# ugonfor/DGQ

Measured on AMD Instinct MI355X. Metric: UNet denoise steps/sec @ SD1.4 512^2 W4A8 g16, higher is better.
Workload: dtype int8 (W4A8 MFMA, int32 accumulate; fp32 between layers); 1 GPU; SD v1.4 UNet W4A8 g=16 (time-aware, log2 softmax real-time δ, start-peak), DDIM 50-step schedule, 512x512 (64x64 latents), CFG pair per step per GPU; config_id=c2, prompts_per_gpu=1, batch_per_gpu=2, parallelism=replicas x1 (no collectives)

## Files before the change

### dgq_amd/csrc/conv_f32w.hip

```cpp
#include "quant_common.h"

typedef float v16f __attribute__((ext_vector_type(16)));

struct ConvF32Params {
    const void* x;
    const float* w;
    const float* bias;
    const float* pre_scale;
    const float* pre_shift;
    int pre_act;
    void* y;
    void* y2;
    int ldy2;
    float* gn_partial;
    int x_dtype, y_dtype;
    int B, H, W, C, kh, kw, stride, pad, Ho, Wo, N, K, M, ldy;
};

__device__ __forceinline__ float ld_any(const void* p, int dtype, int64_t i);
__device__ __forceinline__ float ld_pre(const ConvF32Params& p, int b, int64_t pix, int c) {
    float v = ld_any(p.x, p.x_dtype, pix * p.C + c);
    if (p.pre_scale) v = v * p.pre_scale[(int64_t)b * p.C + c] + p.pre_shift[(int64_t)b * p.C + c];
    if (p.pre_act == 1) v = dgq_silu(v);
    return v;
}

__device__ __forceinline__ void store_any(void* p, int dtype, int64_t i, float v) {
    if (dtype == DGQ_F16) reinterpret_cast<__half*>(p)[i] = __float2half(v);
    else if (dtype == DGQ_BF16) reinterpret_cast<__hip_bfloat16*>(p)[i] = __float2bfloat16(v);
    else reinterpret_cast<float*>(p)[i] = v;
}
__device__ __forceinline__ float ld_any(const void* p, int dtype, int64_t i) {
    if (dtype == DGQ_F16) return __half2float(reinterpret_cast<const __half*>(p)[i]);
    if (dtype == DGQ_BF16) return __bfloat162float(reinterpret_cast<const __hip_bfloat16*>(p)[i]);
    return reinterpret_cast<const float*>(p)[i];
}

#define CF_BM 64
#define CF_BN 64
#define CF_BK 16
#define CF_LD (CF_BK + 1)

__global__ __launch_bounds__(256) void conv_f32w_kernel(ConvF32Params p) {
    __shared__ float As[CF_BM][CF_LD];
    __shared__ float Bs[CF_BN][CF_LD];
    const int tid = threadIdx.x, lane = tid & 63, wid = tid >> 6;
    const int m0 = blockIdx.y * CF_BM, n0 = blockIdx.x * CF_BN;
    const int wm = (wid >> 1) * 32, wn = (wid & 1) * 32;
    const int srow = tid >> 2, sk = (tid & 3) * 4;
    const int am = m0 + srow;
    int ab = 0, aho = 0, awo = 0;
    if (am < p.M) {
        const int L = p.Ho * p.Wo;
        ab = am / L;
        const int l = am - ab * L;
        aho = l / p.Wo;
        awo = l - aho * p.Wo;
    }
    v16f acc;
#pragma unroll
    for (int r = 0; r < 16; ++r) acc[r] = 0.0f;
    for (int k0 = 0; k0 < p.K; k0 += CF_BK) {
#pragma unroll
        for (int j = 0; j < 4; ++j) {
            const int k = k0 + sk + j;
            float a = 0.0f, b = 0.0f;
            if (k < p.K) {
                if (am < p.M) {
                    const int tap = k / p.C, c = k - tap * p.C;
                    const int dh = tap / p.kw, dw = tap - dh * p.kw;
                    const int hi = aho * p.stride - p.pad + dh, wi = awo * p.stride - p.pad + dw;
                    if (hi >= 0 && hi < p.H && wi >= 0 && wi < p.W)
                        a = ld_pre(p, ab, ((int64_t)ab * p.H + hi) * p.W + wi, c);
                }
                if (n0 + srow < p.N) b = p.w[(int64_t)(n0 + srow) * p.K + k];
            }
            As[srow][sk + j] = a;
            Bs[srow][sk + j] = b;
        }
        __syncthreads();
#pragma unroll
        for (int kk = 0; kk < CF_BK; kk += 2) {
            const float av = As[wm + (lane & 31)][kk + (lane >> 5)];
            const float bv = Bs[wn + (lane & 31)][kk + (lane >> 5)];
            acc = __builtin_amdgcn_mfma_f32_32x32x2f32(av, bv, acc, 0, 0, 0);
        }
        __syncthreads();
    }
    const int n = n0 + wn + (lane & 31);
    if (n >= p.N) return;
    const float bias = p.bias ? p.bias[n] : 0.0f;
#pragma unroll
    for (int r = 0; r < 16; ++r) {
        const int m = m0 + wm + (r & 3) + 8 * (r >> 2) + 4 * (lane >> 5);
        if (m >= p.M) continue;
        const float v = acc[r] + bias;
        store_any(p.y, p.y_dtype, (int64_t)m * p.ldy + n, v);
        if (p.y2) store_any(p.y2, p.y_dtype, (int64_t)m * p.ldy2 + n, v);
    }
    if (p.gn_partial) {
#pragma unroll
        for (int blk = 0; blk < 2; ++blk) {
            float val[8], sum = 0.0f;
#pragma unroll
            for (int q = 0; q < 8; ++q) {
                float v = acc[blk * 8 + q] + bias;
                if (p.y_dtype == DGQ_F16) v = __half2float(__float2half(v));
                else if (p.y_dtype == DGQ_BF16) v = __bfloat162float(__float2bfloat16(v));
                val[q] = v;
                sum += v;
            }
            float mean = sum * 0.125f, m2 = 0.0f;
#pragma unroll
            for (int q = 0; q < 8; ++q) m2 += (val[q] - mean) * (val[q] - mean);
            const float om = __shfl_xor(mean, 32, 64), o2 = __shfl_xor(m2, 32, 64);
            const float dd = om - mean;
            m2 = m2 + o2 + dd * dd * 4.0f;
            mean = 0.5f * (mean + om);
            const int mb = m0 + wm + blk * 16;
            if ((lane >> 5) == 0 && mb < p.M) {
                float* q2 = p.gn_partial + ((int64_t)(mb >> 4) * p.N + n) * 2;
                q2[0] = mean; q2[1] = m2;
            }
        }
    }
}

template <int NMAX>
__global__ __launch_bounds__(256) void conv_f32w_smalln_kernel(ConvF32Params p) {
    const int lane = threadIdx.x & 63;
    const int m = blockIdx.x * 4 + (threadIdx.x >> 6);
    if (m >= p.M) return;
    const int L = p.Ho * p.Wo;
    const int b = m / L, l = m - b * L;
    const int ho = l / p.Wo, wo = l - ho * p.Wo;
    float acc[NMAX];
#pragma unroll
    for (int n = 0; n < NMAX; ++n) acc[n] = 0.0f;
    const bool vec = (p.C & 3) == 0 && (reinterpret_cast<uintptr_t>(p.x) & 15) == 0 &&
                     (reinterpret_cast<uintptr_t>(p.w) & 15) == 0 &&
                     (!p.pre_scale || (((reinterpret_cast<uintptr_t>(p.pre_scale) | reinterpret_cast<uintptr_t>(p.pre_shift)) & 15) == 0));
    if (vec) {
        const int c4n = p.C >> 2, units = p.kh * p.kw * c4n;
        constexpr int UB = NMAX <= 4 ? 4 : 2;
        for (int u0 = lane; u0 < units; u0 += 64 * UB) {
            float4 v[UB], sc[UB], sh[UB], w4[UB][NMAX];
            bool inb[UB];
#pragma unroll
            for (int j = 0; j < UB; ++j) {
                const int u = min(u0 + 64 * j, units - 1);
                const int tap = u / c4n, c = (u - tap * c4n) << 2;
                const int dh = tap / p.kw, dw = tap - dh * p.kw;
                const int hi = ho * p.stride - p.pad + dh, wi = wo * p.stride - p.pad + dw;
                inb[j] = (u0 + 64 * j < units) && hi >= 0 && hi < p.H && wi >= 0 && wi < p.W;
                const int hc = min(max(hi, 0), p.H - 1), wc = min(max(wi, 0), p.W - 1);
                const int64_t xi = (((int64_t)b * p.H + hc) * p.W + wc) * p.C + c;
                float t4[4];
                if (p.x_dtype == DGQ_F32) load4<float>(reinterpret_cast<const float*>(p.x) + xi, t4);
                else if (p.x_dtype == DGQ_BF16) load4<__hip_bfloat16>(reinterpret_cast<const __hip_bfloat16*>(p.x) + xi, t4);
                else load4<__half>(reinterpret_cast<const __half*>(p.x) + xi, t4);
                v[j] = make_float4(t4[0], t4[1], t4[2], t4[3]);
                if (p.pre_scale) {
                    sc[j] = *reinterpret_cast<const float4*>(p.pre_scale + (int64_t)b * p.C + c);
                    sh[j] = *reinterpret_cast<const float4*>(p.pre_shift + (int64_t)b * p.C + c);
                }
#pragma unroll
                for (int n = 0; n < NMAX; ++n)
                    if (n < p.N) w4[j][n] = *reinterpret_cast<const float4*>(p.w + (int64_t)n * p.K + (int64_t)tap * p.C + c);
            }
#pragma unroll
            for (int j = 0; j < UB; ++j) {
                float4 t = v[j];
                if (p.pre_scale) {
                    t.x = t.x * sc[j].x + sh[j].x; t.y = t.y * sc[j].y + sh[j].y; t.z = t.z * sc[j].z + sh[j].z; t.w = t.w * sc[j].w + sh[j].w;
                }
                if (p.pre_act == 1) { t.x = dgq_silu(t.x); t.y = dgq_silu(t.y); t.z = dgq_silu(t.z); t.w = dgq_silu(t.w); }
                if (!inb[j]) t = make_float4(0.0f, 0.0f, 0.0f, 0.0f);
#pragma unroll
                for (int n = 0; n < NMAX; ++n)
                    if (n < p.N) {
                        acc[n] = __builtin_fmaf(t.x, w4[j][n].x, acc[n]);
                        acc[n] = __builtin_fmaf(t.y, w4[j][n].y, acc[n]);
                        acc[n] = __builtin_fmaf(t.z, w4[j][n].z, acc[n]);
                        acc[n] = __builtin_fmaf(t.w, w4[j][n].w, acc[n]);
                    }
            }
        }
    } else
    for (int k = lane; k < p.K; k += 64) {
        const int tap = k / p.C, c = k - tap * p.C;
        const int dh = tap / p.kw, dw = tap - dh * p.kw;
        const int hi = ho * p.stride - p.pad + dh, wi = wo * p.stride - p.pad + dw;
        if (hi < 0 || hi >= p.H || wi < 0 || wi >= p.W) continue;
        const float a = ld_pre(p, b, ((int64_t)b * p.H + hi) * p.W + wi, c);
#pragma unroll
        for (int n = 0; n < NMAX; ++n)
            if (n < p.N) acc[n] = __builtin_fmaf(a, p.w[(int64_t)n * p.K + k], acc[n]);
    }
#pragma unroll
    for (int n = 0; n < NMAX; ++n) {
        float v = acc[n];
#pragma unroll
        for (int o = 32; o > 0; o >>= 1) v += __shfl_xor(v, o, 64);
        if (lane == 0 && n < p.N) {
            v += p.bias ? p.bias[n] : 0.0f;
            store_any(p.y, p.y_dtype, (int64_t)m * p.ldy + n, v);
            if (p.y2) store_any(p.y2, p.y_dtype, (int64_t)m * p.ldy2 + n, v);
        }
    }
}

extern "C" int dgq_conv2d_f32w(const void* x, int x_dtype, int B, int H, int W, int C, int kh, int kw, int stride, int pad,
                               const float* w, const float* bias, int N, void* y, int y_dtype, int ldy,
                               const float* pre_scale, const float* pre_shift, int pre_act, void* y2, int ldy2, float* gn_partial, void* stream) {
    DGQ_CHECK_ARG(x && w && y, "dgq_conv2d_f32w: null pointer");
    DGQ_CHECK_ARG(B > 0 && H > 0 && W > 0 && C > 0 && kh > 0 && kw > 0 && stride > 0 && pad >= 0 && N > 0, "dgq_conv2d_f32w: bad geometry");
    DGQ_CHECK_ARG((x_dtype == DGQ_F32 || x_dtype == DGQ_F16 || x_dtype == DGQ_BF16) && (y_dtype == DGQ_F32 || y_dtype == DGQ_F16 || y_dtype == DGQ_BF16),
                  "dgq_conv2d_f32w: unknown dtype");
    DGQ_CHECK_ARG((pre_scale == nullptr) == (pre_shift == nullptr) && (pre_act == 0 || pre_act == 1), "dgq_conv2d_f32w: bad prologue");
    ConvF32Params p;
    p.pre_scale = pre_scale; p.pre_shift = pre_shift; p.pre_act = pre_act;
    p.x = x; p.w = w; p.bias = bias; p.y = y; p.x_dtype = x_dtype; p.y_dtype = y_dtype;
    p.B = B; p.H = H; p.W = W; p.C = C; p.kh = kh; p.kw = kw; p.stride = stride; p.pad = pad;
    p.Ho = (H + 2 * pad - kh) / stride + 1; p.Wo = (W + 2 * pad - kw) / stride + 1;
    DGQ_CHECK_ARG(p.Ho > 0 && p.Wo > 0, "dgq_conv2d_f32w: empty output");
    p.N = N; p.K = kh * kw * C; p.M = B * p.Ho * p.Wo; p.ldy = ldy;
    DGQ_CHECK_ARG(ldy >= N && (!y2 || ldy2 >= N), "dgq_conv2d_f32w: ldy < N");
    p.y2 = y2; p.ldy2 = ldy2;
    DGQ_CHECK_ARG(!gn_partial || (p.M % 16 == 0 && N > 8), "dgq_conv2d_f32w: GroupNorm partials need M %% 16 == 0 and the tiled kernel (N > 8)");
    p.gn_partial = gn_partial;
    if (N <= 8) {
        if (N <= 4) hipLaunchKernelGGL(conv_f32w_smalln_kernel<4>, dim3((p.M + 3) / 4), dim3(256), 0, (hipStream_t)stream, p);
        else hipLaunchKernelGGL(conv_f32w_smalln_kernel<8>, dim3((p.M + 3) / 4), dim3(256), 0, (hipStream_t)stream, p);
        return dgq_launch_status("dgq_conv2d_f32w");
    }
    dim3 grid((N + CF_BN - 1) / CF_BN, (p.M + CF_BM - 1) / CF_BM);
    DGQ_CHECK_ARG(grid.y <= 65535, "dgq_conv2d_f32w: M = %d rows exceed the grid", p.M);
    hipLaunchKernelGGL(conv_f32w_kernel, grid, dim3(256), 0, (hipStream_t)stream, p);
    return dgq_launch_status("dgq_conv2d_f32w");
}
```

### dgq_amd/csrc/gemm_tile.h

```cpp
#pragma once
#include <atomic>
#include <cstdio>
#include <cstdlib>
#include <type_traits>
#include "dgq_common.h"
#include "gemm_device.h"
#include "gemm_flush.h"
#include "diag.h"

#define BK 128

typedef int v16i __attribute__((ext_vector_type(16)));
typedef float v16f __attribute__((ext_vector_type(16)));

struct GemmParams {
    const int8_t* codes;
    const float* rowsum;
    int rowsum_parts;
    int M, Kp, N;
    const uint8_t* wpacked;
    const float* cdelta;
    const uint8_t* cflush;
    const float* mdelta;
    const float* mzp;
    int L;
    float offset;
    const float* alpha;
    const float* zw;
    const float* gamma;
    const float* vn;
    void* y;
    int ldy;
    float* slab;
    int splits;
    int tiles_per_split;
    dgq_gemm_extra_t ex;
    dgq_gemm_conv_t cv;
    const float* ccoef;
    const uint8_t* wfrag;
    dgq_gemm_act_t act;
};

#define DGQ_GEMM_BATCH 8
struct GemmBatch {
    GemmParams p[DGQ_GEMM_BATCH];
    int n;
};

__device__ __forceinline__ void gemm_prefetch_params(const GemmParams& p) {
    asm volatile("" ::"s"(p.M), "s"(p.N), "s"(p.Kp), "s"(p.tiles_per_split), "s"(p.splits), "s"(p.codes), "s"(p.wpacked), "s"(p.rowsum),
                 "s"(p.rowsum_parts), "s"(p.alpha), "s"(p.zw), "s"(p.gamma), "s"(p.vn), "s"(p.cdelta), "s"(p.cflush), "s"(p.mdelta),
                 "s"(p.mzp), "s"(p.L), "s"(p.offset), "s"(p.y), "s"(p.ldy), "s"(p.slab), "s"(p.ex.residual), "s"(p.ex.ldr),
                 "s"(p.ex.res_div), "s"(p.ex.res_dtype), "s"(p.ex.fq_mode), "s"(p.ex.geglu), "s"(p.ex.gn_partial), "s"(p.wfrag), "s"(p.ex.y2));
}

template <bool PER_M>
__device__ __forceinline__ float dgq_epilogue(const GemmParams& p, float acc, int m, int n, float al, float zw, float ga,
                                              float vn) {
    float rs = 0.0f;
    for (int j = 0; j < p.rowsum_parts; ++j) rs += p.rowsum[(int64_t)j * p.M + m];
    if (PER_M) {
        const int li = m % p.L;
        const float md = p.mdelta[li], mz = p.mzp[li];
        return dgq_dequant<true>(acc, md, md * rs, md * (p.offset - mz), al, zw, ga, vn);
    }
    return dgq_dequant<false>(acc, 1.0f, rs, 0.0f, al, zw, ga, vn);
}

constexpr int gemm_stage_bytes(int wbits, int bm, int bn) { return bm * BK + bn * (wbits == 4 ? BK / 2 : BK); }
constexpr int gemm_waves_per_simd(int wbits, int bm, int bn, int nw, int nst) {
    const int per_block = nst * gemm_stage_bytes(wbits, bm, bn) + 6 * 1024;
    int o = (160 * 1024) / per_block;
    o = o > 5 ? 5 : (o < 1 ? 1 : o);
    const int w = o * nw / 4;
    return w > 8 ? 8 : w;
}

__device__ __forceinline__ float gload_f32(const float* q) {
    float v;
    asm volatile("global_load_dword %0, %1, off" : "=v"(v) : "v"(q) : "memory");
    return v;
}
__device__ __forceinline__ uint32_t gload_u8(const uint8_t* q) {
    uint32_t v;
    asm volatile("global_load_ubyte %0, %1, off" : "=v"(v) : "v"(q) : "memory");
    return v;
}
template <int N>
__device__ __forceinline__ void wait_vmcnt_lgkm0() {
    asm volatile("s_waitcnt vmcnt(%0) lgkmcnt(0)" ::"n"(N) : "memory");
}
template <int PER, int MAXT>
__device__ __forceinline__ void wait_ring(int tiles) {
    static_assert(PER * MAXT <= 63, "vmcnt is a 6-bit counter");
    if (tiles <= 0) wait_vmcnt_lgkm0<0>();
    else if (MAXT >= 1 && tiles == 1) wait_vmcnt_lgkm0<PER>();
    else if (MAXT >= 2 && tiles == 2) wait_vmcnt_lgkm0<PER * (MAXT >= 2 ? 2 : 0)>();
    else if (MAXT >= 3 && tiles == 3) wait_vmcnt_lgkm0<PER * (MAXT >= 3 ? 3 : 0)>();
    else wait_vmcnt_lgkm0<PER * (MAXT >= 4 ? 4 : 0)>();
}

struct GemmColRegs { float al, zw, ga, vn; };
template <bool PER_M>
__device__ __forceinline__ GemmColRegs gemm_cols_issue(const GemmParams& p, int n) {
    GemmColRegs c;
    c.al = gload_f32(p.alpha + n); c.zw = gload_f32(p.zw + n); c.ga = gload_f32(p.gamma + n);
    c.vn = 0.0f;
    if constexpr (PER_M) c.vn = gload_f32(p.vn + n);
    return c;
}
template <bool PER_M, int BN>
__device__ __forceinline__ void gemm_cols_commit(GemmColRegs& c, float* vcol, int tid, bool has_col) {
    if (PER_M) asm volatile("" : "+v"(c.al), "+v"(c.zw), "+v"(c.ga), "+v"(c.vn));
    else asm volatile("" : "+v"(c.al), "+v"(c.zw), "+v"(c.ga));
    __builtin_amdgcn_sched_barrier(0);
    if (has_col) {
        vcol[tid] = c.al; vcol[BN + tid] = c.zw; vcol[2 * BN + tid] = c.ga; vcol[3 * BN + tid] = c.vn;
    }
}
struct GemmFlushRegs { FlushRef x; float d, dn; uint32_t cf; };
template <typename Ref>
__device__ __forceinline__ GemmFlushRegs gemm_flush_issue(const GemmParams& p, int n_tab, int tid, Ref&& ref) {
    GemmFlushRegs f;
    f.x = ref(min(tid, n_tab - 1));
    f.d = gload_f32(p.cdelta + f.x.g); f.dn = gload_f32(p.cdelta + f.x.gn); f.cf = gload_u8(p.cflush + f.x.tl);
    return f;
}
template <int NT, typename Ref>
__device__ __forceinline__ void gemm_flush_commit(const GemmParams& p, GemmFlushRegs& f, float* ctab, int n_tab, int tid, Ref&& ref) {
    asm volatile("" : "+v"(f.d), "+v"(f.dn), "+v"(f.cf));
    __builtin_amdgcn_sched_barrier(0);
    if (tid < n_tab) ctab[tid] = flush_value(f.x, f.d, f.dn, f.cf);
    for (int e = tid + NT; e < n_tab; e += NT) ctab[e] = flush_entry(ref(e), p.cdelta, p.cflush);
}

template <bool BIASED, int TM, int TN>
__device__ __forceinline__ void gemm_flush(v16f (&accf)[TM][TN], const v16i (&ac)[TM][TN], float coef) {
    const float sc = __builtin_bit_cast(float, __builtin_amdgcn_readfirstlane(__builtin_bit_cast(int, coef)));
    if (sc != 0.0f) {
#pragma unroll
        for (int i = 0; i < TM; ++i)
#pragma unroll
            for (int j = 0; j < TN; ++j)
#pragma unroll
                for (int r = 0; r < 16; ++r) accf[i][j][r] = __builtin_fmaf(sc, dgq_total_to_float<BIASED>(ac[i][j][r]), accf[i][j][r]);
    }
}
template <int ACC0, int ACCS, int TM, int TN>
__device__ __forceinline__ void gemm_clear_totals(v16i (&acc)[ACCS][TM][TN]) {
#pragma unroll
    for (int a = 0; a < ACCS; ++a)
#pragma unroll
        for (int i = 0; i < TM; ++i)
#pragma unroll
            for (int j = 0; j < TN; ++j)
#pragma unroll
                for (int r = 0; r < 16; ++r) acc[a][i][j][r] = ACC0;
}


template <bool PER_M, typename TOut, int BM, int BN, int WVM, int WVN, int WVK, int LDS_CAP, int TM, int TN, bool TILED = false>
__device__ __forceinline__ void gemm_store_tile(const GemmParams& p, int zsplit, uint8_t* smem, const float* vtab, const float* vcol,
                                                int wid, int lane, int wave_m, int wave_n, int wave_k, int m0, int n0,
                                                const v16i (&acc0)[TM][TN], const v16f (&accf)[TM][TN] DGQ_DIAG_PARAM,
                                                int tiled_w = 0, int tiled_gn0 = 0) {
    static_assert(!TILED || (BM == 32 && WVM == 1 && WVK == 1), "tiled rows: one 32-row tile per workgroup");
    constexpr int NW = WVM * WVN * WVK;
    constexpr int WM = BM / WVM, WN = BN / WVN;
    static_assert(TM == WM / 32 && TN == WN / 32, "wave tile");
    const int lr = lane & 31, hh = lane >> 5;
    constexpr int EP_LD = WN + 4;
    constexpr int LPR = WN / 4;
    constexpr int RPP = 64 / LPR;
    constexpr int PASSES = WM / RPP / WVK;
    constexpr int EPH = (NW * WM * EP_LD * 4 <= LDS_CAP) ? 1 : 2;
    static_assert(EPH == 1 || (WVK == 1 && TM % 2 == 0 && PASSES % 2 == 0), "half-tile staging: whole MFMA row tiles per half");
    constexpr int HROWS = WM / EPH;
    constexpr int REGION = HROWS * EP_LD;
    static_assert(NW * REGION * 4 <= LDS_CAP, "epilogue staging must fit the LDS ring");
    float* ep_all = reinterpret_cast<float*>(smem);
    float* ep = ep_all + wid * REGION;
    auto stage_half = [&](int h) {
#pragma unroll
        for (int i = 0; i < TM / EPH; ++i)
#pragma unroll
            for (int j = 0; j < TN; ++j)
#pragma unroll
                for (int r = 0; r < 16; ++r) {
                    const int ti = h * (TM / EPH) + i;
                    ep[(i * 32 + (r & 3) + 8 * (r >> 2) + 4 * hh) * EP_LD + j * 32 + lr] = PER_M ? (float)acc0[ti][j][r] : accf[ti][j][r];
                }
        asm volatile("s_waitcnt lgkmcnt(0)" ::: "memory");
    };
    auto next_half = [&](int rr) {
        if (EPH == 2 && rr == PASSES / 2) {
            asm volatile("s_waitcnt lgkmcnt(0)" ::: "memory");
            stage_half(1);
        }
    };
    stage_half(0);
    if (WVK > 1) __builtin_amdgcn_s_barrier();
    DGQ_STAMP(8);
    const float* ep0 = ep_all + (wave_m * WVN + wave_n) * REGION;
    const float* ep1 = ep0 + (WVM * WVN) * REGION;
    const int c4 = (lane % LPR) * 4;
    const int lrow = lane / LPR;
    const int nb = n0 + wave_n * WN + c4;
    const bool vec_ok = (nb + 3 < p.N);
    auto tile_row = [&](int rr) { return wave_k * (WM / WVK) + rr * RPP + lrow; };
    auto row_m = [&](int row) { return TILED ? m0 + (row >> 3) * tiled_w + (row & 7) : m0 + wave_m * WM + row; };
    auto tile_val = [&](int row) {
        const int sr = (EPH == 2) ? (row & (HROWS - 1)) : row;
        float4 v = *reinterpret_cast<const float4*>(ep0 + sr * EP_LD + c4);
        if (WVK > 1) {
            const float4 u = *reinterpret_cast<const float4*>(ep1 + sr * EP_LD + c4);
            v.x += u.x; v.y += u.y; v.z += u.z; v.w += u.w;
        }
        return v;
    };
    if (p.splits > 1) {
        float* slab = p.slab + (int64_t)zsplit * p.M * p.N;
        const bool al16 = ((p.N & 3) == 0);
#pragma unroll 4
        for (int rr = 0; rr < PASSES; ++rr) {
            next_half(rr);
            const int row = tile_row(rr);
            const int m = row_m(row);
            if (m >= p.M || nb >= p.N) continue;
            const float4 v = tile_val(row);
            float* dst = slab + (int64_t)m * p.N + nb;
            if (vec_ok && al16) {
                *reinterpret_cast<float4*>(dst) = v;
            } else {
                const float e[4] = {v.x, v.y, v.z, v.w};
                for (int k = 0; k < 4 && nb + k < p.N; ++k) dst[k] = e[k];
            }
        }
        return;
    }
    TOut* y = reinterpret_cast<TOut*>(p.y);
    const float* vc = vcol + wave_n * WN + c4;
    const float4 al = *reinterpret_cast<const float4*>(vc);
    const float4 zw = *reinterpret_cast<const float4*>(vc + BN);
    const float4 ga = *reinterpret_cast<const float4*>(vc + 2 * BN);
    const float4 vn = *reinterpret_cast<const float4*>(vc + 3 * BN);
    if (p.ex.geglu) {
        const int ob = nb >> 1;
        const bool st2 = vec_ok && (p.ldy % 2 == 0) && ((reinterpret_cast<uintptr_t>(p.y) & 7) == 0);
#pragma unroll
        for (int rr = 0; rr < PASSES; ++rr) {
            next_half(rr);
            const int row = tile_row(rr);
            const int m = row_m(row);
            if (m >= p.M || nb >= p.N) continue;
            const float4 v = tile_val(row);
            const float* vr = vtab + wave_m * WM + row;
            const float r0 = vr[0], r1 = vr[BM], r2 = vr[2 * BM];
            const float a0 = dgq_dequant<PER_M>(v.x, r0, r1, r2, al.x, zw.x, ga.x, vn.x);
            const float g0 = dgq_dequant<PER_M>(v.y, r0, r1, r2, al.y, zw.y, ga.y, vn.y);
            const float a1 = dgq_dequant<PER_M>(v.z, r0, r1, r2, al.z, zw.z, ga.z, vn.z);
            const float g1 = dgq_dequant<PER_M>(v.w, r0, r1, r2, al.w, zw.w, ga.w, vn.w);
            const float o0 = dgq_geglu(a0, g0), o1 = dgq_geglu(a1, g1);
            TOut* dst = y + (int64_t)m * p.ldy + ob;
            if (st2) {
                if (sizeof(TOut) == 4) {
                    *reinterpret_cast<float2*>(dst) = make_float2(o0, o1);
                } else {
                    TOut t[2] = {dgq_from_float<TOut>(o0), dgq_from_float<TOut>(o1)};
                    *reinterpret_cast<uint32_t*>(dst) = *reinterpret_cast<const uint32_t*>(t);
                }
            } else {
                dst[0] = dgq_from_float<TOut>(o0);
                if (nb + 3 < p.N) dst[1] = dgq_from_float<TOut>(o1);
            }
        }
        return;
    }
    const bool st_vec = vec_ok && ((p.ldy * (int)sizeof(TOut)) % 16 == 0) &&
                        ((reinterpret_cast<uintptr_t>(p.y) & 15) == 0) && (sizeof(TOut) == 4 || (p.ldy & 3) == 0);
    const bool st_vec2 = vec_ok && ((p.ex.ldy2 * (int)sizeof(TOut)) % 16 == 0) &&
                         ((reinterpret_cast<uintptr_t>(p.ex.y2) & 15) == 0) && (sizeof(TOut) == 4 || (p.ex.ldy2 & 3) == 0);
    const int res_es = p.ex.res_dtype == DGQ_F32 ? 4 : 2;
    const bool res_vec = p.ex.residual != nullptr && vec_ok && (p.ex.ldr & 3) == 0 &&
                         (reinterpret_cast<uintptr_t>(p.ex.residual) & (4 * res_es - 1)) == 0;
    constexpr int HP = PASSES / EPH;
    float4 res[HP];
    auto load_res = [&](int h) {
        if (!res_vec) return;
#pragma unroll
        for (int q = 0; q < HP; ++q) {
            const int m = min(row_m(tile_row(h * HP + q)), p.M - 1);
            const int64_t i = (int64_t)(m / p.ex.res_div) * p.ex.ldr + nb;
            if (p.ex.res_dtype == DGQ_F32) {
                res[q] = *reinterpret_cast<const float4*>(reinterpret_cast<const float*>(p.ex.residual) + i);
            } else {
                const uint2 t = *reinterpret_cast<const uint2*>(reinterpret_cast<const uint16_t*>(p.ex.residual) + i);
                if (p.ex.res_dtype == DGQ_F16) {
                    const __half* h16 = reinterpret_cast<const __half*>(&t);
                    res[q] = make_float4(__half2float(h16[0]), __half2float(h16[1]), __half2float(h16[2]), __half2float(h16[3]));
                } else {
                    res[q] = make_float4(__uint_as_float(t.x << 16), __uint_as_float(t.x & 0xFFFF0000u),
                                         __uint_as_float(t.y << 16), __uint_as_float(t.y & 0xFFFF0000u));
                }
            }
        }
    };
    load_res(0);
    dgq_gemm_extra_t exl = p.ex;
    if (res_vec) exl.residual = nullptr;
    const bool has_extra = exl.fq_mode != 0 || exl.residual != nullptr;
    constexpr int PPB = (16 / RPP) < 1 ? 1 : (16 / RPP);
    static_assert(RPP <= 16 && (WM / WVK) % 16 == 0, "GroupNorm partials: 16-row blocks per wave");
    const bool gn = p.ex.gn_partial != nullptr;
    float gK[4] = {0.f, 0.f, 0.f, 0.f}, g1[4] = {0.f, 0.f, 0.f, 0.f}, g2[4] = {0.f, 0.f, 0.f, 0.f};
#pragma unroll
    for (int rr = 0; rr < PASSES; ++rr) {
        next_half(rr);
        if (EPH == 2 && rr == HP) load_res(1);
        const int row = tile_row(rr);
        const int m = row_m(row);
        if (m >= p.M || nb >= p.N) continue;
        const float4 v = tile_val(row);
        const float* vr = vtab + wave_m * WM + row;
        const float r0 = vr[0], r1 = vr[BM], r2 = vr[2 * BM];
        float o[4];
        o[0] = dgq_dequant<PER_M>(v.x, r0, r1, r2, al.x, zw.x, ga.x, vn.x);
        o[1] = dgq_dequant<PER_M>(v.y, r0, r1, r2, al.y, zw.y, ga.y, vn.y);
        o[2] = dgq_dequant<PER_M>(v.z, r0, r1, r2, al.z, zw.z, ga.z, vn.z);
        o[3] = dgq_dequant<PER_M>(v.w, r0, r1, r2, al.w, zw.w, ga.w, vn.w);
        if (has_extra) {
#pragma unroll
            for (int k = 0; k < 4; ++k)
                if (nb + k < p.N) o[k] = dgq_extra(exl, o[k], m, nb + k);
        }
        if (res_vec) {
            o[0] += res[rr % HP].x; o[1] += res[rr % HP].y; o[2] += res[rr % HP].z; o[3] += res[rr % HP].w;
        }
#pragma unroll
        for (int cp = 0; cp < 2; ++cp) {
            if (cp == 1 && p.ex.y2 == nullptr) break;
            TOut* dst = cp == 0 ? y + (int64_t)m * p.ldy + nb : reinterpret_cast<TOut*>(p.ex.y2) + (int64_t)m * p.ex.ldy2 + nb;
            if (cp == 0 ? st_vec : st_vec2) {
                if (sizeof(TOut) == 4) {
                    *reinterpret_cast<float4*>(dst) = make_float4(o[0], o[1], o[2], o[3]);
                } else {
                    TOut t[4] = {dgq_from_float<TOut>(o[0]), dgq_from_float<TOut>(o[1]), dgq_from_float<TOut>(o[2]),
                                 dgq_from_float<TOut>(o[3])};
                    *reinterpret_cast<uint2*>(dst) = *reinterpret_cast<const uint2*>(t);
                }
            } else {
                for (int k = 0; k < 4 && nb + k < p.N; ++k) dst[k] = dgq_from_float<TOut>(o[k]);
            }
        }
        if (gn) {
#pragma unroll
            for (int k = 0; k < 4; ++k) {
                const float val = dgq_to_float(dgq_from_float<TOut>(o[k]));
                if (rr % PPB == 0) { gK[k] = val; g1[k] = 0.0f; g2[k] = 0.0f; }
                else { const float dv = val - gK[k]; g1[k] += dv; g2[k] += dv * dv; }
            }
            if (rr % PPB == PPB - 1) {
                float mean[4], m2[4];
#pragma unroll
                for (int k = 0; k < 4; ++k) {
                    const float md = g1[k] * (1.0f / PPB);
                    mean[k] = gK[k] + md;
                    m2[k] = fmaxf(g2[k] - g1[k] * md, 0.0f);
                }
                float cnt = (float)PPB;
#pragma unroll
                for (int off = LPR; off < 64; off <<= 1) {
#pragma unroll
                    for (int k = 0; k < 4; ++k) {
                        const float om = __shfl_xor(mean[k], off, 64), o2 = __shfl_xor(m2[k], off, 64);
                        const float dd = om - mean[k];
                        m2[k] = m2[k] + o2 + dd * dd * (0.5f * cnt);
                        mean[k] = 0.5f * (mean[k] + om);
                    }
                    cnt *= 2.0f;
                }
                if (lrow == 0) {
                    float* q = p.ex.gn_partial + ((int64_t)(TILED ? tiled_gn0 + (row >> 4) : (m >> 4)) * p.N + nb) * 2;
                    *reinterpret_cast<float4*>(q) = make_float4(mean[0], m2[0], mean[1], m2[1]);
                    *reinterpret_cast<float4*>(q + 4) = make_float4(mean[2], m2[2], mean[3], m2[3]);
                }
            }
        }
    }
}
```

### dgq_amd/csrc/gemm_wxa8.hip

```cpp
#include "gemm_tile.h"
#include "quant_common.h"

DGQ_DIAG_BUFFER(gemm)

template <int WBITS, bool PER_M, typename TOut, int BM, int BN, int WVM, int WVN, int WVK, int NST, int ACCS, bool CONV = false>
__global__ __launch_bounds__(64 * WVM * WVN * WVK, gemm_waves_per_simd(WBITS, BM, BN, WVM * WVN * WVK, NST))
void gemm_wxa8_kernel(GemmBatch bt) {
    const GemmParams& p = bt.p[bt.n > 1 ? blockIdx.z : 0];
    const int zsplit = bt.n > 1 ? 0 : blockIdx.z;
    gemm_prefetch_params(p);
    int tile_n, tile_m;
    {
        const int gx = gridDim.x;
        const int logical = dgq_xcd_logical(blockIdx.x + gx * blockIdx.y, gx * gridDim.y);
        tile_m = logical / gx;
        tile_n = logical - tile_m * gx;
    }
    if (tile_n * BN >= p.N || tile_m * BM >= p.M) return;
    DGQ_DIAG_DECL
    DGQ_STAMP(0); DGQ_STAMP_REAL(1); DGQ_STAMP_WHERE(2);
    extern __shared__ __attribute__((aligned(16))) uint8_t smem[];
    constexpr int STAGES = NST;
    constexpr int NW = WVM * WVN * WVK, NT = 64 * NW;
    constexpr int WM = BM / WVM, WN = BN / WVN;
    static_assert(WM % 32 == 0 && WN % 32 == 0, "wave tile: multiples of the 32x32 MFMA tile");
    constexpr int TM = WM / 32, TN = WN / 32;
    constexpr int MYCH = NCH / WVK;
    static_assert(WVK == 1 || WVK == 2, "K split inside the workgroup: 1 or 2");
    static_assert(ACCS == 1 || (ACCS == 2 && !PER_M), "two accumulator sets: per-K mode only");
    static_assert(NST >= 3 && NST <= 6, "ring depth");
    constexpr int A_BYTES = BM * BK;
    constexpr int W_ROW = (WBITS == 4) ? BK / 2 : BK;
    constexpr int W_BYTES = BN * W_ROW;
    constexpr int STAGE_BYTES = A_BYTES + W_BYTES;
    static_assert(A_BYTES % (1024 * NW) == 0 && W_BYTES % (1024 * NW) == 0, "every wave stages whole 1-KiB pieces of each operand");
    constexpr int A_DMA = A_BYTES / 1024 / NW;
    constexpr int W_DMA = W_BYTES / 1024 / NW;
    constexpr int DMA_PER_TILE = A_DMA + W_DMA;

    const int tid = threadIdx.x;
    const int lane = tid & 63;
    const int wid = __builtin_amdgcn_readfirstlane(tid >> 6);
    const int wave_k = wid / (WVM * WVN), wave_m = (wid / WVN) % WVM, wave_n = wid % WVN;
    const int n0 = tile_n * BN;
    const int m0 = tile_m * BM;
    const int nk_total = p.Kp / BK;
    const int kt_begin = zsplit * p.tiles_per_split;
    const int kt_end = min(nk_total, kt_begin + p.tiles_per_split);
    const int nk = kt_end - kt_begin;

    const int8_t* a_src[A_DMA];
    int cv_cc[A_DMA], cv_dh[A_DMA], cv_dw[A_DMA], cv_k[A_DMA], cv_h[A_DMA], cv_w[A_DMA];
    const int8_t* cv_img[A_DMA];
    bool cv_in[A_DMA];
#pragma unroll
    for (int i = 0; i < A_DMA; ++i) {
        const int blk = wid * A_DMA + i;
        const int row = blk * 8 + (lane >> 3);
        const int c = (lane & 7) ^ ((row >> 1) & 7);
        const int m = min(m0 + row, p.M - 1);
        if constexpr (CONV) {
            const int L = p.cv.Ho * p.cv.Wo;
            const int b = m / L, l = m - b * L;
            const int ho = l / p.cv.Wo, wo = l - ho * p.cv.Wo;
            cv_h[i] = ho * p.cv.stride - p.cv.pad;
            cv_w[i] = wo * p.cv.stride - p.cv.pad;
            a_src[i] = p.cv.codes_in + (int64_t)b * p.cv.H * p.cv.W * p.cv.ldc;
            const int k = kt_begin * BK + 16 * c;
            const int tap = k / p.cv.C;
            cv_k[i] = k;
            cv_cc[i] = k - tap * p.cv.C;
            cv_dh[i] = tap / p.cv.kw;
            cv_dw[i] = tap - cv_dh[i] * p.cv.kw;
            cv_img[i] = a_src[i];
            const int hi = cv_h[i] + cv_dh[i], wi = cv_w[i] + cv_dw[i];
            cv_in[i] = (unsigned)hi < (unsigned)p.cv.H && (unsigned)wi < (unsigned)p.cv.W;
            a_src[i] = cv_img[i] + ((int64_t)hi * p.cv.W + wi) * p.cv.ldc + cv_cc[i];
        } else {
            a_src[i] = p.codes + (int64_t)m * p.Kp + 16 * c;
        }
    }
    const uint8_t* w_src[W_DMA];
#pragma unroll
    for (int i = 0; i < W_DMA; ++i) {
        const int blk = wid * W_DMA + i;
        if (WBITS == 4) {
            const int row = blk * 16 + (lane >> 2);
            const int c = (lane & 3) ^ ((row >> 2) & 3);
            const int n = min(n0 + row, p.N - 1);
            w_src[i] = p.wpacked + (int64_t)n * (p.Kp / 2) + 16 * c;
        } else {
            const int row = blk * 8 + (lane >> 3);
            const int c = (lane & 7) ^ ((row >> 1) & 7);
            const int n = min(n0 + row, p.N - 1);
            w_src[i] = p.wpacked + (int64_t)n * p.Kp + 16 * c;
        }
    }

    const uint32_t lds_base = (uint32_t)(uintptr_t)(lptr_t)smem;
    auto issue_tile = [&](int kt, int stage) {
        const uint32_t sa = lds_base + stage * STAGE_BYTES;
        const uint32_t sw = sa + A_BYTES;
        const int64_t ka = (int64_t)kt * BK;
        const int64_t kw = (WBITS == 4) ? ka / 2 : ka;
#pragma unroll
        for (int i = 0; i < A_DMA; ++i) {
            if constexpr (CONV) {
                const int8_t* src = cv_in[i] ? a_src[i] : p.cv.fill;
                if (cv_k[i] >= p.cv.C * p.cv.kh * p.cv.kw) src = p.cv.fill + 16;
                glds16(src, __builtin_amdgcn_readfirstlane(sa + (wid * A_DMA + i) * 1024));
                cv_k[i] += BK;
                cv_cc[i] += BK;
                a_src[i] += BK;
                if (__builtin_expect(__any(cv_cc[i] >= p.cv.C), 0)) {
                    if (cv_cc[i] >= p.cv.C) {
                        const int tap = cv_k[i] / p.cv.C;
                        cv_cc[i] = cv_k[i] - tap * p.cv.C;
                        cv_dh[i] = tap / p.cv.kw;
                        cv_dw[i] = tap - cv_dh[i] * p.cv.kw;
                        const int hi = cv_h[i] + cv_dh[i], wi = cv_w[i] + cv_dw[i];
                        cv_in[i] = (unsigned)hi < (unsigned)p.cv.H && (unsigned)wi < (unsigned)p.cv.W;
                        a_src[i] = cv_img[i] + ((int64_t)hi * p.cv.W + wi) * p.cv.ldc + cv_cc[i];
                    }
                }
            } else {
                glds16(a_src[i] + ka, __builtin_amdgcn_readfirstlane(sa + (wid * A_DMA + i) * 1024));
            }
        }
#pragma unroll
        for (int i = 0; i < W_DMA; ++i)
            glds16(w_src[i] + kw, __builtin_amdgcn_readfirstlane(sw + (wid * W_DMA + i) * 1024));
    };

    v16i acc[ACCS][TM][TN];
    v16f accf[TM][TN];
    constexpr bool BIASED = !PER_M && WBITS == 4;
    constexpr int ACC0 = BIASED ? DGQ_ACC_BIAS_I : 0;
#pragma unroll
    for (int i = 0; i < TM; ++i)
#pragma unroll
        for (int j = 0; j < TN; ++j) {
#pragma unroll
            for (int r = 0; r < 16; ++r) {
#pragma unroll
                for (int a = 0; a < ACCS; ++a) acc[a][i][j][r] = ACC0;
                accf[i][j][r] = 0.0f;
            }
        }

    const int lr = lane & 31, hh = lane >> 5;
    int a_off[TM][MYCH], w_off[TN][MYCH];
#pragma unroll
    for (int ci = 0; ci < MYCH; ++ci) {
        const int cg = ci * WVK + wave_k;
#pragma unroll
        for (int i = 0; i < TM; ++i) {
            const int row = wave_m * WM + i * 32 + lr;
            a_off[i][ci] = row * BK + (((2 * cg + hh) ^ ((row >> 1) & 7)) << 4);
        }
#pragma unroll
        for (int j = 0; j < TN; ++j) {
            const int row = wave_n * WN + j * 32 + lr;
            if (WBITS == 4) w_off[j][ci] = row * W_ROW + ((cg ^ ((row >> 2) & 3)) << 4) + ((hh ^ ((row >> 4) & 1)) << 3);
            else w_off[j][ci] = row * BK + (((2 * cg + hh) ^ ((row >> 1) & 7)) << 4);
        }
    }

    float* vtab = reinterpret_cast<float*>(smem + STAGES * STAGE_BYTES);
    float* vcol = vtab + 3 * BM;
    float* ctab = vcol + 4 * BN;
    static_assert(BM <= NT && BN <= NT, "one row / column of the epilogue vectors per thread");
    const int per_wave = nk * MYCH, n_coef = PER_M ? 0 : WVK * per_wave, n_tab = PER_M ? 0 : n_coef + nk;
    const FlushGeom fg = {ACCS * WVK, kt_begin, nk, nk_total, 0};
    auto tab_ref = [&](int e) {
        const int ec = e < n_coef ? e : 0;
        const int kq = ec / per_wave, i = ec - kq * per_wave;
        const int tc = i / MYCH, ci = i - tc * MYCH;
        return flush_ref(fg, e < n_coef, (kt_begin + tc) * NCH + ci * WVK + kq, e - n_coef);
    };
    {
        const bool final_ep = (p.splits == 1);
        const bool has_row = final_ep && tid < BM, has_col = final_ep && tid < BN;
        const int m = min(m0 + tid, p.M - 1), n = min(n0 + tid, p.N - 1);
        const int li = PER_M ? m % p.L : 0;
        float md = 1.0f, mz = 0.0f;
        float rs = gload_f32(p.rowsum + m);
        if constexpr (PER_M) { md = gload_f32(p.mdelta + li); mz = gload_f32(p.mzp + li); }
        GemmColRegs cr = gemm_cols_issue<PER_M>(p, n);
        GemmFlushRegs fr = {};
        if constexpr (!PER_M) fr = gemm_flush_issue(p, n_tab, tid, tab_ref);
        int issued = 0;
#pragma unroll
        for (int i = 0; i < STAGES - 1; ++i)
            if (i < nk) { issue_tile(kt_begin + i, i); ++issued; }
        DGQ_STAMP(3);
        wait_ring<DMA_PER_TILE, STAGES - 2>(issued - 1);
        DGQ_STAMP(4);
        if (PER_M) asm volatile("" : "+v"(rs), "+v"(md), "+v"(mz));
        else asm volatile("" : "+v"(rs));
        __builtin_amdgcn_sched_barrier(0);
        if (has_row) {
            for (int j = 1; j < p.rowsum_parts; ++j) rs += p.rowsum[(int64_t)j * p.M + m];
            float r0 = 1.0f, r1 = rs, r2 = 0.0f;
            if (PER_M) { r0 = md; r1 = md * rs; r2 = md * (p.offset - mz); }
            vtab[tid] = r0; vtab[BM + tid] = r1; vtab[2 * BM + tid] = r2;
        }
        gemm_cols_commit<PER_M, BN>(cr, vcol, tid, has_col);
        if constexpr (!PER_M) gemm_flush_commit<NT>(p, fr, ctab, n_tab, tid, tab_ref);
    }
    asm volatile("s_waitcnt lgkmcnt(0)" ::: "memory");
    __builtin_amdgcn_s_barrier();

    typedef typename std::conditional<WBITS == 4, uint2, v4i>::type wfrag_t;
    auto load_frags = [&](const uint8_t* sa, const uint8_t* sw, int ci, v4i (&af)[TM], wfrag_t (&wf)[TN]) {
#pragma unroll
        for (int i = 0; i < TM; ++i) af[i] = *reinterpret_cast<const v4i*>(sa + a_off[i][ci]);
#pragma unroll
        for (int j = 0; j < TN; ++j) wf[j] = *reinterpret_cast<const wfrag_t*>(sw + w_off[j][ci]);
    };
    const float* ctw = ctab + wave_k * (nk * MYCH);
    const float* tclr = ctab + WVK * (nk * MYCH);
    typedef float cvec_t __attribute__((ext_vector_type(MYCH)));
    auto mfma_chunk = [&](const v4i (&af)[TM], const wfrag_t (&wf)[TN], v16i (&ac)[TM][TN]) {
        v4i bf[TN];
#pragma unroll
        for (int j = 0; j < TN; ++j) {
            if constexpr (WBITS == 4) {
                const uint2 v = wf[j];
                bf[j] = (v4i){(int)(v.x & 0x0F0F0F0Fu), (int)((v.x >> 4) & 0x0F0F0F0Fu),
                              (int)(v.y & 0x0F0F0F0Fu), (int)((v.y >> 4) & 0x0F0F0F0Fu)};
            } else {
                bf[j] = wf[j];
            }
        }
#pragma unroll
        for (int i = 0; i < TM; ++i)
#pragma unroll
            for (int j = 0; j < TN; ++j)
                ac[i][j] = __builtin_amdgcn_mfma_i32_32x32x32_i8(af[i], bf[j], ac[i][j], 0, 0, 0);
    };
    auto flush = [&](const v16i (&ac)[TM][TN], float coef) { gemm_flush<BIASED>(accf, ac, coef); };
    float pend = 0.0f;
    auto step = [&](const v4i (&af)[TM], const wfrag_t (&wf)[TN], int ci, float coef) {
        if constexpr (PER_M) {
            mfma_chunk(af, wf, acc[0]);
        } else if constexpr (ACCS == 1) {
            mfma_chunk(af, wf, acc[0]);
            flush(acc[0], coef);
        } else {
            if (ci & 1) { mfma_chunk(af, wf, acc[1]); flush(acc[0], pend); }
            else { mfma_chunk(af, wf, acc[0]); flush(acc[1], pend); }
            pend = coef;
        }
    };
    v4i af0[TM], af1[TM];
    wfrag_t wf0[TN], wf1[TN];
    int stage = 0, istage = STAGES - 1;
    DGQ_STAMP(5);
    load_frags(smem, smem + A_BYTES, 0, af0, wf0);
    for (int t = 0; t < nk; ++t) {
        if (t + STAGES - 1 < nk) issue_tile(kt_begin + t + STAGES - 1, istage);
        cvec_t cq;
        float tc = 0.0f;
        if (!PER_M) {
            cq = *reinterpret_cast<const cvec_t*>(ctw + t * MYCH);
            tc = tclr[t];
            __builtin_amdgcn_sched_barrier(0);
        }
        const uint8_t* sa = smem + stage * STAGE_BYTES;
#pragma unroll
        for (int ci = 0; ci + 1 < MYCH; ++ci) {
            if ((ci & 1) == 0) {
                load_frags(sa, sa + A_BYTES, ci + 1, af1, wf1);
                step(af0, wf0, ci, PER_M ? 0.0f : cq[ci]);
            } else {
                load_frags(sa, sa + A_BYTES, ci + 1, af0, wf0);
                step(af1, wf1, ci, PER_M ? 0.0f : cq[ci]);
            }
        }
        DGQ_STAMP_NOW(dg_w0);
        wait_ring<DMA_PER_TILE, STAGES - 2>(min(STAGES - 2, nk - 2 - t));
        DGQ_STAMP_ACC(12, dg_w0);
        __builtin_amdgcn_s_barrier();
        DGQ_STAMP_ACC(7, dg_w0);
        stage = (stage + 1 == STAGES) ? 0 : stage + 1;
        istage = (istage + 1 == STAGES) ? 0 : istage + 1;
        if (t + 1 < nk) {
            const uint8_t* sn = smem + stage * STAGE_BYTES;
            load_frags(sn, sn + A_BYTES, 0, af0, wf0);
        }
        step(af1, wf1, MYCH - 1, PER_M ? 0.0f : cq[MYCH - 1]);
        if (!PER_M) {
            if (__builtin_amdgcn_readfirstlane(__builtin_bit_cast(int, tc)) != 0) {
                if constexpr (ACCS == 2) { flush(acc[1], pend); pend = 0.0f; }
                gemm_clear_totals<ACC0>(acc);
            }
        }
    }
    if constexpr (!PER_M && ACCS == 2) flush(acc[1], pend);
    DGQ_STAMP(6);

    gemm_store_tile<PER_M, TOut, BM, BN, WVM, WVN, WVK, STAGES * STAGE_BYTES, TM, TN>(p, zsplit, smem, vtab, vcol, wid, lane, wave_m, wave_n,
                                                                                      wave_k, m0, n0, acc[0], accf DGQ_DIAG_ARG);
    DGQ_STAMP(9);
    DGQ_DIAG_DRAIN();
    DGQ_STAMP(10); DGQ_STAMP_REAL(11);
#ifdef DGQ_DIAG
    dg.t[13] = (unsigned long long)nk | ((unsigned long long)tile_m << 16) | ((unsigned long long)tile_n << 32) | ((unsigned long long)wid << 48);
#endif
    DGQ_DIAG_FLUSH(gemm, NW, wid, lane);
}

template <int R>
__device__ __forceinline__ void splitk_sum_slabs(const float* base, int64_t slab_stride, int splits, float (&a)[4]) {
    for (int s0 = 0; s0 < splits; s0 += R) {
        float4 v[R];
#pragma unroll
        for (int j = 0; j < R; ++j) v[j] = *reinterpret_cast<const float4*>(base + (int64_t)min(s0 + j, splits - 1) * slab_stride);
#pragma unroll
        for (int j = 0; j < R; ++j)
            if (s0 + j < splits) { a[0] += v[j].x; a[1] += v[j].y; a[2] += v[j].z; a[3] += v[j].w; }
    }
}
__device__ __forceinline__ void splitk_sum(const float* base, int64_t slab_stride, int splits, float (&a)[4]) {
    if (splits <= 4) splitk_sum_slabs<4>(base, slab_stride, splits, a);
    else if (splits <= 8) splitk_sum_slabs<8>(base, slab_stride, splits, a);
    else splitk_sum_slabs<16>(base, slab_stride, splits, a);
}

template <bool PER_M, typename TOut>
__global__ __launch_bounds__(256) void splitk_epilogue_kernel(GemmParams p) {
    const int n4 = (p.N + 3) / 4;
    TOut* y = reinterpret_cast<TOut*>(p.y);
    const int64_t slab_stride = (int64_t)p.M * p.N;
    const bool vec4 = ((p.N & 3) == 0) && ((p.ldy * (int)sizeof(TOut)) % 16 == 0) && ((reinterpret_cast<uintptr_t>(p.y) & 15) == 0) &&
                      (p.ex.y2 == nullptr || (((p.ex.ldy2 * (int)sizeof(TOut)) % 16 == 0) && (reinterpret_cast<uintptr_t>(p.ex.y2) & 15) == 0)) &&
                      p.ex.fq_mode == 0 && !p.ex.geglu &&
                      (((reinterpret_cast<uintptr_t>(p.alpha) | reinterpret_cast<uintptr_t>(p.zw) | reinterpret_cast<uintptr_t>(p.gamma) |
                         (PER_M ? reinterpret_cast<uintptr_t>(p.vn) : 0)) & 15) == 0) &&
                      (p.ex.residual == nullptr || ((p.ex.ldr & 3) == 0 && (reinterpret_cast<uintptr_t>(p.ex.residual) & (p.ex.res_dtype == DGQ_F32 ? 15 : 7)) == 0));
    auto row4 = [&](int m, int nb, float (&val)[4], bool live) {
        float a[4] = {0.f, 0.f, 0.f, 0.f};
        const bool full = (nb + 3 < p.N) && ((p.N & 3) == 0);
        if (full) {
            splitk_sum(p.slab + (int64_t)m * p.N + nb, slab_stride, p.splits, a);
        } else {
            for (int s = 0; s < p.splits; ++s) {
                const float* src = p.slab + s * slab_stride + (int64_t)m * p.N + nb;
                for (int e = 0; e < 4 && nb + e < p.N; ++e) a[e] += src[e];
            }
        }
        if (full && vec4) {
            const float4 al = *reinterpret_cast<const float4*>(p.alpha + nb), zw = *reinterpret_cast<const float4*>(p.zw + nb);
            const float4 ga = *reinterpret_cast<const float4*>(p.gamma + nb);
            const float4 vn = PER_M ? *reinterpret_cast<const float4*>(p.vn + nb) : make_float4(0.f, 0.f, 0.f, 0.f);
            float rs = 0.0f;
            for (int j = 0; j < p.rowsum_parts; ++j) rs += p.rowsum[(int64_t)j * p.M + m];
            float r0 = 1.0f, r1 = rs, r2 = 0.0f;
            if (PER_M) {
                const int li = m % p.L;
                const float md = p.mdelta[li], mz = p.mzp[li];
                r0 = md; r1 = md * rs; r2 = md * (p.offset - mz);
            }
            float o[4];
            o[0] = dgq_dequant<PER_M>(a[0], r0, r1, r2, al.x, zw.x, ga.x, vn.x);
            o[1] = dgq_dequant<PER_M>(a[1], r0, r1, r2, al.y, zw.y, ga.y, vn.y);
            o[2] = dgq_dequant<PER_M>(a[2], r0, r1, r2, al.z, zw.z, ga.z, vn.z);
            o[3] = dgq_dequant<PER_M>(a[3], r0, r1, r2, al.w, zw.w, ga.w, vn.w);
            if (p.ex.residual) {
                const int64_t ri = (int64_t)(m / p.ex.res_div) * p.ex.ldr + nb;
                float r[4];
                if (p.ex.res_dtype == DGQ_F32) load4<float>(reinterpret_cast<const float*>(p.ex.residual) + ri, r);
                else if (p.ex.res_dtype == DGQ_BF16) load4<__hip_bfloat16>(reinterpret_cast<const __hip_bfloat16*>(p.ex.residual) + ri, r);
                else load4<__half>(reinterpret_cast<const __half*>(p.ex.residual) + ri, r);
                o[0] += r[0]; o[1] += r[1]; o[2] += r[2]; o[3] += r[3];
            }
            TOut* dst = y + (int64_t)m * p.ldy + nb;
            TOut* dst2 = p.ex.y2 ? reinterpret_cast<TOut*>(p.ex.y2) + (int64_t)m * p.ex.ldy2 + nb : nullptr;
            if (sizeof(TOut) == 4) {
                if (live) *reinterpret_cast<float4*>(dst) = make_float4(o[0], o[1], o[2], o[3]);
                if (live && dst2) *reinterpret_cast<float4*>(dst2) = make_float4(o[0], o[1], o[2], o[3]);
#pragma unroll
                for (int e = 0; e < 4; ++e) val[e] = o[e];
            } else {
                TOut t[4] = {dgq_from_float<TOut>(o[0]), dgq_from_float<TOut>(o[1]), dgq_from_float<TOut>(o[2]), dgq_from_float<TOut>(o[3])};
                if (live) *reinterpret_cast<uint2*>(dst) = *reinterpret_cast<const uint2*>(t);
                if (live && dst2) *reinterpret_cast<uint2*>(dst2) = *reinterpret_cast<const uint2*>(t);
#pragma unroll
                for (int e = 0; e < 4; ++e) val[e] = dgq_to_float(t[e]);
            }
            return;
        }
        for (int e = 0; e < 4 && nb + e < p.N; ++e) {
            const int n = nb + e;
            float out = dgq_epilogue<PER_M>(p, a[e], m, n, p.alpha[n], p.zw[n], p.gamma[n], PER_M ? p.vn[n] : 0.0f);
            out = dgq_extra(p.ex, out, m, n);
            const TOut st = dgq_from_float<TOut>(out);
            if (live) y[(int64_t)m * p.ldy + n] = st;
            if (live && p.ex.y2) reinterpret_cast<TOut*>(p.ex.y2)[(int64_t)m * p.ex.ldy2 + n] = st;
            val[e] = dgq_to_float(st);
        }
    };
    if (p.ex.gn_partial) {
        const int64_t units = (int64_t)(p.M >> 4) * n4;
        const int64_t tid = (int64_t)blockIdx.x * blockDim.x + threadIdx.x;
        const int lane = (int)(tid & 63);
        const int qd = lane >> 2;
        const int64_t unit = (tid >> 6) * 4 + (lane & 3);
        const bool live = unit < units;
        const int64_t g = live ? unit : units - 1;
        const int rb = (int)(g / n4);
        const int nb = (int)(g - (int64_t)rb * n4) * 4;
        const int m = rb * 16 + qd;
        float mean[4], m2[4] = {0.f, 0.f, 0.f, 0.f};
        row4(m, nb, mean, live);
        float cnt = 1.0f;
#pragma unroll
        for (int off = 4; off < 64; off <<= 1) {
#pragma unroll
            for (int e = 0; e < 4; ++e) {
                const float om = __shfl_xor(mean[e], off, 64), o2 = __shfl_xor(m2[e], off, 64);
                const float dd = om - mean[e];
                m2[e] = m2[e] + o2 + dd * dd * (0.5f * cnt);
                mean[e] = 0.5f * (mean[e] + om);
            }
            cnt *= 2.0f;
        }
        if (live && qd == 0) {
            float* q = p.ex.gn_partial + ((int64_t)rb * p.N + nb) * 2;
            *reinterpret_cast<float4*>(q) = make_float4(mean[0], m2[0], mean[1], m2[1]);
            *reinterpret_cast<float4*>(q + 4) = make_float4(mean[2], m2[2], mean[3], m2[3]);
        }
        return;
    }
    const int64_t total = (int64_t)p.M * n4;
    for (int64_t i = (int64_t)blockIdx.x * blockDim.x + threadIdx.x; i < total; i += (int64_t)gridDim.x * blockDim.x) {
        const int m = (int)(i / n4);
        float val[4];
        row4(m, (int)(i - (int64_t)m * n4) * 4, val, true);
    }
}

int dgq_launch_gemm_big(const GemmBatch& bt, bool per_m, int y_dtype, hipStream_t st);
size_t dgq_gemm_big_lds_bytes(bool per_m, int Kp);
int dgq_launch_gemm_panel(const GemmBatch& bt, bool per_m, int y_dtype, int nw, int kw, hipStream_t st);
size_t dgq_gemm_panel_lds_bytes(int nw, int kw, bool per_m, int tiles);
int dgq_gemm_convq_plan(int B, int H, int W, int C, int kh, int kw, int stride, int pad, int N, int Kp, int w_bits, bool per_m, int* lds_bytes);
int dgq_launch_gemm_convq(const GemmBatch& bt, bool per_m, int y_dtype, int slab_tiles, int lds, hipStream_t st);

template <bool PER_M, typename TOut>
static void launch_combine(const GemmParams& p, hipStream_t st);
enum class GemmKind { Tile, Rows256, Panel };
struct GemmPlan { int bm, bn, splits; double t; int kw = 1; bool fuse = false; GemmKind kind = GemmKind::Tile; };
static GemmPlan plan_rows256() { GemmPlan pl = {256, 256, 1, 0.0}; pl.kind = GemmKind::Rows256; return pl; }

template <int WBITS, bool PER_M, typename TOut, int BM, int BN, int WVM, int WVN, int WVK, int NST>
static void launch_tile(const GemmBatch& bt, hipStream_t st) {
    const GemmParams& p = bt.p[0];
    constexpr int NW = WVM * WVN * WVK;
    constexpr int ACCS = (!PER_M && (BM / WVM / 32) * (BN / WVN / 32) <= 2) ? 2 : 1;
    constexpr int lds_stages = NST * gemm_stage_bytes(WBITS, BM, BN);
    constexpr int lds_vec = (3 * BM + 4 * BN) * 4;
    constexpr int lds_max = lds_stages + lds_vec + 32768;
    static std::atomic<bool> attr_set[64];
    dgq_allow_dynamic_lds(attr_set, {{&gemm_wxa8_kernel<WBITS, PER_M, TOut, BM, BN, WVM, WVN, WVK, NST, ACCS>, lds_max}});
    int maxN = 0, maxM = 0, max_tps = 0;
    for (int i = 0; i < bt.n; ++i) {
        maxN = bt.p[i].N > maxN ? bt.p[i].N : maxN;
        maxM = bt.p[i].M > maxM ? bt.p[i].M : maxM;
        max_tps = bt.p[i].tiles_per_split > max_tps ? bt.p[i].tiles_per_split : max_tps;
    }
    const int lds = lds_stages + lds_vec + (PER_M ? 0 : (((NCH + 1) * max_tps * 4 + 15) & ~15));
    dim3 grid((maxN + BN - 1) / BN, (maxM + BM - 1) / BM, bt.n > 1 ? bt.n : p.splits), block(64 * NW);
    if (p.cv.codes_in) {
        if constexpr (WBITS == 4 && PER_M && ((BM == 32 && BN == 64) || (BM == 64 && BN == 64) || (BM == 64 && BN == 128) || (BM == 128 && BN == 128))) {
            static std::atomic<bool> cattr[64];
            dgq_allow_dynamic_lds(cattr, {{&gemm_wxa8_kernel<WBITS, PER_M, TOut, BM, BN, WVM, WVN, WVK, NST, ACCS, true>, lds_max}});
            hipLaunchKernelGGL((gemm_wxa8_kernel<WBITS, PER_M, TOut, BM, BN, WVM, WVN, WVK, NST, ACCS, true>), grid, block, lds, st, bt);
        }
        return;
    }
    hipLaunchKernelGGL((gemm_wxa8_kernel<WBITS, PER_M, TOut, BM, BN, WVM, WVN, WVK, NST, ACCS>), grid, block, lds, st, bt);
}

template <int WBITS, bool PER_M, typename TOut, int BM, int BN, int WVM, int WVN, int WVK>
static void launch_ring(const GemmBatch& bt, hipStream_t st) {
    launch_tile<WBITS, PER_M, TOut, BM, BN, WVM, WVN, WVK, 3>(bt, st);
}

template <int WBITS, bool PER_M, typename TOut>
static int launch_one(const GemmBatch& bt, int bm, int bn, hipStream_t st) {
    const GemmParams& p = bt.p[0];
    const int key = bm * 1000 + bn;
    switch (key) {
        case 128128: launch_ring<WBITS, PER_M, TOut, 128, 128, 2, 2, 1>(bt, st); break;
        case 64064: launch_ring<WBITS, PER_M, TOut, 64, 64, 2, 2, 1>(bt, st); break;
        case 32064: launch_ring<WBITS, PER_M, TOut, 32, 64, 1, 2, 2>(bt, st); break;
        default:
            if constexpr (WBITS == 4) {
                switch (key) {
                    case 128064: launch_ring<WBITS, PER_M, TOut, 128, 64, 2, 2, 1>(bt, st); break;
                    case 64128: launch_ring<WBITS, PER_M, TOut, 64, 128, 1, 4, 1>(bt, st); break;
                    case 32128: launch_ring<WBITS, PER_M, TOut, 32, 128, 1, 4, 1>(bt, st); break;
                    default: dgq_set_error("dgq_gemm_wxa8: no %dx%d tile", bm, bn); return DGQ_EINVAL;
                }
            } else {
                dgq_set_error("dgq_gemm_wxa8: no %dx%d tile for W8", bm, bn);
                return DGQ_EINVAL;
            }
    }
    if (bt.n == 1 && p.splits > 1) launch_combine<PER_M, TOut>(p, st);
    return DGQ_OK;
}

template <bool PER_M, typename TOut>
static void launch_combine(const GemmParams& p, hipStream_t st) {
    int64_t total = (int64_t)p.M * ((p.N + 3) / 4);
    if (p.ex.gn_partial) total = ((int64_t)(p.M / 16) * ((p.N + 3) / 4) + 3) / 4 * 64;
    int g = (int)((total + 255) / 256);
    if (g > 4096 && !p.ex.gn_partial) g = 4096;
    hipLaunchKernelGGL((splitk_epilogue_kernel<PER_M, TOut>), dim3(g), dim3(256), 0, st, p);
}

template <int WBITS, bool PER_M>
static int launch_gemm(const GemmBatch& p, const GemmPlan& pl, int y_dtype, hipStream_t st) {
    const int bm = pl.bm, bn = pl.bn;
    int rc;
    if (pl.kind == GemmKind::Rows256) {
        DGQ_CHECK_ARG(WBITS == 4 && p.n == 1 && p.p[0].splits == 1 && dgq_gemm_big_lds_bytes(PER_M, p.p[0].Kp) <= 160 * 1024,
                      "dgq_gemm_wxa8: the 256-row kernel takes one unsplit W4 problem whose tables fit the LDS");
        rc = dgq_launch_gemm_big(p, PER_M, y_dtype, st);
        if (rc != DGQ_OK) return rc;
        return dgq_launch_status("dgq_gemm_wxa8");
    }
    if (pl.kind == GemmKind::Panel) {
        const int tm = bm / 32, nw = bn / 32;
        DGQ_CHECK_ARG(WBITS == 4 && pl.fuse, "dgq_gemm_wxa8: the panel kernel is the quantise-on-load form of W4 layers");
        for (int i = 0; i < p.n; ++i) {
            DGQ_CHECK_ARG(p.p[i].wfrag && !p.p[i].cv.codes_in && p.p[i].act.x, "dgq_gemm_wxa8: quantise-on-load needs the fragment-major weights (extra.wfrag) and the activation descriptor (extra.act)");
            const size_t need = tm == 1 ? dgq_gemm_panel_lds_bytes(nw, pl.kw, PER_M, p.p[i].tiles_per_split) : 0;
            DGQ_CHECK_ARG(need > 0 && need <= 160 * 1024, "dgq_gemm_wxa8: no panel configuration TM=%d NW=%d KW=%d for a K extent of %d tiles",
                          tm, nw, pl.kw, p.p[i].tiles_per_split);
            DGQ_CHECK_ARG(p.p[i].splits == 1, "dgq_gemm_wxa8: quantise-on-load takes the whole K extent in one workgroup");
        }
        rc = dgq_launch_gemm_panel(p, PER_M, y_dtype, nw, pl.kw, st);
        if (rc != DGQ_OK) return rc;
        return dgq_launch_status("dgq_gemm_wxa8");
    }
    switch (y_dtype) {
        case DGQ_F32: rc = launch_one<WBITS, PER_M, float>(p, bm, bn, st); break;
        case DGQ_F16: rc = launch_one<WBITS, PER_M, __half>(p, bm, bn, st); break;
        case DGQ_BF16: rc = launch_one<WBITS, PER_M, __hip_bfloat16>(p, bm, bn, st); break;
        default: dgq_set_error("dgq_gemm_wxa8: unknown y dtype %d", y_dtype); return DGQ_EINVAL;
    }
    if (rc != DGQ_OK) return rc;
    return dgq_launch_status("dgq_gemm_wxa8");
}

static GemmPlan plan_gemm(int M, int N, int Kp, int w_bits, size_t ws_bytes, bool per_m, bool allow_big = true) {
    const int nk = Kp / BK;
    const double out = (double)M * N;
    GemmPlan pl = {32, 64, 1, 0.0};
    if (out > 3.0e7) {
        pl = {128, 128, 1, 0.0};
    } else if (out > 3.0e6) {
        pl = {64, 128, 1, 0.0};
    } else if (nk > 60) {
        if (M <= 160) pl = {32, 64, 1, 0.0};
        else if (N >= 1280) pl = (M >= 2048) ? GemmPlan{64, 64, 1, 0.0} : GemmPlan{128, 64, 1, 0.0};
        else if (M >= 4096 && N % 128 != 0) pl = {64, 64, 1, 0.0};
        else pl = {64, 128, 1, 0.0};
        const long grid = (long)((M + pl.bm - 1) / pl.bm) * ((N + pl.bn - 1) / pl.bn);
        if (grid < 256) {
            int s = (int)((480 + grid - 1) / grid);
            if (s > nk / 8) s = nk / 8;
            if (s > 16) s = 16;
            while (s > 1 && (double)s * out * 4.0 > (double)ws_bytes) --s;
            pl.splits = s < 1 ? 1 : s;
        }
    } else if (M >= 4096 && nk >= 24) {
        pl = (N % 128 != 0) ? GemmPlan{64, 64, 1, 0.0} : GemmPlan{32, 128, 1, 0.0};
    }
    {
        const int bn_big = per_m ? 256 : 128;
        const long tiles = (long)((M + 255) / 256) * ((N + bn_big - 1) / bn_big);
        constexpr long min_tiles = 256;
        if (allow_big && w_bits == 4 && pl.splits == 1 && M >= 2048 && N % bn_big == 0 && tiles >= min_tiles &&
            (nk >= 32 || (per_m && nk >= 8 && N >= 4096)) && dgq_gemm_big_lds_bytes(per_m, Kp) <= 160 * 1024)
            pl = plan_rows256();
    }
    if (w_bits != 4) {
        if (pl.bm == 128 || pl.bn == 128) { pl.bm = 128; pl.bn = 128; }
        else if (pl.bm == 64) { pl.bm = 64; pl.bn = 64; }
        else { pl.bm = 32; pl.bn = 64; }
    }
    return pl;
}

static bool plan_panel_fuse(int M, int N, int Kp, bool per_m, GemmPlan& pl) {
    static const bool on = [] { const char* e = getenv("DGQ_GEMM_FUSE"); return !(e && *e == '0'); }();
    if (!on) return false;
    const int nk = Kp / BK;
    const long mb = (M + 31) / 32, nt = (N + 31) / 32;
    const int kw = (mb * nt < 2048 && nk >= 4) ? 2 : 1;
    int nw;
    if (kw == 1) nw = (N % 320 == 0) ? 10 : 5;
    else nw = (N % 160 == 0) ? 5 : 4;
    const size_t need = dgq_gemm_panel_lds_bytes(nw, kw, per_m, nk);
    if (need == 0 || need > 150 * 1024) return false;
    const char* ea = getenv("DGQ_GEMM_FUSE_ALL");
    const bool all = ea && *ea == '1';
    if (!all && ((N + 32 * nw - 1) / (32 * nw) > 2 || M < 2048)) return false;
    pl.kind = GemmKind::Panel; pl.bm = 32; pl.bn = 32 * nw; pl.kw = kw; pl.fuse = true; pl.splits = 1;
    return true;
}

extern "C" int dgq_gemm_act_fuses(int M, int N, int K, int Kp, int w_bits, int per_m, int n_problems, int x_dtype, int y_dtype) {
    if (w_bits != 4 || x_dtype != y_dtype || M < 1 || N < 1 || K < 4 || K % 4 != 0 || Kp < K || Kp % BK != 0 || n_problems < 1 || n_problems > DGQ_GEMM_BATCH)
        return 0;
    GemmPlan pl = {32, 64, 1, 0.0};
    return plan_panel_fuse(M, N, Kp, per_m != 0, pl) ? 1 : 0;
}

extern "C" int dgq_gemm_conv_act_fuses(int B, int H, int W, int C, int kh, int kw, int stride, int pad, int N, int Kp, int w_bits, int per_m,
                                       int x_dtype, int y_dtype) {
    static const bool on = [] { const char* e = getenv("DGQ_GEMM_FUSE"); return !(e && *e == '0'); }();
    if (!on || x_dtype != y_dtype) return 0;
    return dgq_gemm_convq_plan(B, H, W, C, kh, kw, stride, pad, N, Kp, w_bits, per_m != 0, nullptr) > 0 ? 1 : 0;
}

static void conv_tile(GemmPlan& pl, int M) {
    const int key = pl.bm * 1000 + pl.bn;
    pl.kind = GemmKind::Tile;
    if (M >= 2048) { pl.bm = 64; pl.bn = 128; return; }
    if (key == 32064 || key == 64064 || key == 64128 || key == 128128) return;
    if (pl.bm >= 128) { pl.bm = 128; pl.bn = 128; }
    else if (pl.bn >= 128) { pl.bm = 64; pl.bn = 128; }
    else { pl.bm = 64; pl.bn = 64; }
}

__global__ __launch_bounds__(256) void conv_rowsum_kernel(dgq_gemm_conv_t c, int M, float* rowsum) {
    const int m = blockIdx.x * blockDim.x + threadIdx.x;
    if (m >= M) return;
    const int L = c.Ho * c.Wo;
    const int b = m / L, l = m - b * L;
    const int ho = l / c.Wo, wo = l - ho * c.Wo;
    const int64_t npix = (int64_t)c.B * c.H * c.W;
    const float* ps = c.pixsum + (int64_t)b * c.H * c.W;
    const float outside = (float)c.C * c.zero_code;
    float s = 0.0f;
    for (int dh = 0; dh < c.kh; ++dh)
        for (int dw = 0; dw < c.kw; ++dw) {
            const int hi = ho * c.stride - c.pad + dh, wi = wo * c.stride - c.pad + dw;
            if ((unsigned)hi < (unsigned)c.H && (unsigned)wi < (unsigned)c.W) {
                for (int q = 0; q < c.pixsum_parts; ++q) s += ps[q * npix + hi * c.W + wi];
            } else {
                s += outside;
            }
        }
    rowsum[m] = s;
}

static bool forced_plan(GemmPlan& pl) {
    const char* e = getenv("DGQ_GEMM_FORCE");
    if (!e || !*e) return false;
    int bm = 0, bn = 0, s = 0;
    if (*e == 'F') {
        int kw = 1;
        if (sscanf(e + 1, "%d,%d,%d,%d", &bm, &bn, &s, &kw) < 3) return false;
        bm *= 32; bn *= 32;
        pl.kind = GemmKind::Panel;
        pl.kw = kw < 1 ? 1 : kw;
        pl.fuse = true;
    } else if (sscanf(e, "%d,%d,%d", &bm, &bn, &s) != 3) {
        return false;
    } else {
        pl.kind = bm == 256 ? GemmKind::Rows256 : GemmKind::Tile;
        pl.fuse = false;
    }
    pl.bm = bm; pl.bn = bn; pl.splits = s < 1 ? 1 : s;
    return true;
}

extern "C" int dgq_gemm_plan_splits(int M, int N, int Kp, int w_bits, int per_m, size_t workspace_bytes) {
    GemmPlan pl = plan_gemm(M, N, Kp, w_bits, workspace_bytes, per_m != 0);
    forced_plan(pl);
    const int nk = Kp / BK;
    if (pl.splits < 1) pl.splits = 1;
    const int tps = (nk + pl.splits - 1) / pl.splits;
    return (nk + tps - 1) / tps;
}

extern "C" size_t dgq_gemm_workspace_bytes(int M, int N, int Kp) {
    const GemmPlan a = plan_gemm(M, N, Kp, 4, (size_t)-1, false), b = plan_gemm(M, N, Kp, 4, (size_t)-1, true);
    const int s = a.splits > b.splits ? a.splits : b.splits;
    return s > 1 ? (size_t)s * M * N * sizeof(float) : 0;
}

static int fill_gemm(const dgq_gemm_args_t& a, GemmParams& p) {
    DGQ_CHECK_ARG(a.codes && a.rowsum && a.wpacked && a.alpha && a.zw && a.gamma && a.y, "dgq_gemm_wxa8: null pointer");
    DGQ_CHECK_ARG(a.M > 0 && a.N > 0 && a.Kp > 0 && a.Kp % DGQ_KTILE == 0, "dgq_gemm_wxa8: bad shape M=%d N=%d Kp=%d", a.M, a.N, a.Kp);
    DGQ_CHECK_ARG(a.w_bits == 4 || a.w_bits == 8, "dgq_gemm_wxa8: w_bits=%d unsupported", a.w_bits);
    DGQ_CHECK_ARG(a.rowsum_parts >= 1 && a.rowsum_parts <= 64, "dgq_gemm_wxa8: rowsum_parts=%d", a.rowsum_parts);
    DGQ_CHECK_ARG(a.ldy >= (a.extra && a.extra->geglu ? a.N / 2 : a.N), "dgq_gemm_wxa8: ldy < output columns");
    DGQ_CHECK_ARG(a.Kp / DGQ_KCHUNK <= 4096 && (!a.per_m || a.Kp <= (a.w_bits == 4 ? 1 << 20 : 1 << 17)),
                  "dgq_gemm_wxa8: Kp=%d too large for W%d", a.Kp, a.w_bits);
    DGQ_CHECK_ARG((reinterpret_cast<uintptr_t>(a.codes) & 15) == 0 && (reinterpret_cast<uintptr_t>(a.wpacked) & 15) == 0,
                  "dgq_gemm_wxa8: codes/wpacked must be 16-byte aligned");
    if (a.per_m) {
        DGQ_CHECK_ARG(a.mdelta && a.mzp && a.vn && a.L >= 1, "dgq_gemm_wxa8: per_m needs mdelta/mzp/vn/L");
    } else {
        DGQ_CHECK_ARG(a.cdelta && a.cflush, "dgq_gemm_wxa8: per-K mode needs cdelta/cflush");
    }
    p.cv.codes_in = nullptr;
    p.ccoef = nullptr;
    p.wfrag = nullptr;
    p.act.x = nullptr;
    p.codes = a.codes; p.rowsum = a.rowsum; p.rowsum_parts = a.rowsum_parts; p.M = a.M; p.Kp = a.Kp; p.N = a.N;
    p.wpacked = reinterpret_cast<const uint8_t*>(a.wpacked);
    p.cdelta = a.cdelta; p.cflush = a.cflush; p.mdelta = a.mdelta; p.mzp = a.mzp; p.L = a.per_m ? a.L : 1; p.offset = a.offset;
    p.alpha = a.alpha; p.zw = a.zw; p.gamma = a.gamma; p.vn = a.vn; p.y = a.y; p.ldy = a.ldy;
    if (a.extra) {
        p.ex = *a.extra;
        DGQ_CHECK_ARG(p.ex.fq_mode >= 0 && p.ex.fq_mode <= 3, "dgq_gemm_wxa8: bad fq_mode");
        DGQ_CHECK_ARG(p.ex.fq_mode == 0 || (p.ex.fq_delta && p.ex.fq_zp && p.ex.fq_T > 0 && p.ex.fq_D > 0), "dgq_gemm_wxa8: fused quantizer needs tables");
        DGQ_CHECK_ARG(!p.ex.residual || (p.ex.ldr >= a.N && p.ex.res_div >= 1 && p.ex.res_dtype >= DGQ_F32 && p.ex.res_dtype <= DGQ_BF16),
                      "dgq_gemm_wxa8: bad residual descriptor (ldr < N, res_div < 1 or unknown dtype)");
        DGQ_CHECK_ARG(!p.ex.geglu || (a.N % 4 == 0 && !p.ex.residual && p.ex.fq_mode == 0),
                      "dgq_gemm_wxa8: the GEGLU epilogue needs N %% 4 == 0 and no other extra");
        if (p.ex.wfrag) {
            DGQ_CHECK_ARG(a.w_bits == 4 && (reinterpret_cast<uintptr_t>(p.ex.wfrag) & 15) == 0, "dgq_gemm_wxa8: wfrag is the W4 layout-2 image, 16-byte aligned");
            p.wfrag = reinterpret_cast<const uint8_t*>(p.ex.wfrag);
        }
        if (p.ex.act) {
            const dgq_gemm_act_t& q = *p.ex.act;
            DGQ_CHECK_ARG(q.x && p.ex.wfrag && q.K > 0 && q.K % 4 == 0 && q.K <= a.Kp && q.ldx >= q.K && q.bits >= 2 && q.bits <= 8 &&
                          q.x_dtype == a.y_dtype && (a.per_m || (q.czp && (q.kh > 1 || q.kdst))) && (q.pre_scale == nullptr) == (q.pre_shift == nullptr) &&
                          (q.kh <= 1 || (q.kpat && !q.ln_gamma && q.B >= 1 && q.H >= 1 && q.W >= 1 && q.kw >= 1 && q.stride >= 1 && q.pad >= 0)) &&
                          (!q.pre_scale || q.rows_per_image >= 1) && (q.pre_act == 0 || q.pre_act == 1) &&
                          (q.ln_gamma == nullptr) == (q.ln_beta == nullptr) && (!q.ln_gamma || (q.ln_eps > 0.0f && !q.pre_scale && q.pre_act == 0)) &&
                          (reinterpret_cast<uintptr_t>(q.x) & 15) == 0 && (q.ldx * (q.x_dtype == DGQ_F32 ? 4 : 2)) % 8 == 0,
                          "dgq_gemm_wxa8: bad quantise-on-load descriptor (needs wfrag, x of the output dtype, K %% 4 == 0, per-K: kdst + czp)");
            p.act = q;
        }
        if (p.ex.flush_coef && !a.per_m) {
            DGQ_CHECK_ARG((reinterpret_cast<uintptr_t>(p.ex.flush_coef) & 15) == 0, "dgq_gemm_wxa8: flush_coef must be 16-byte aligned");
            p.ccoef = p.ex.flush_coef;
        }
        if (p.ex.conv) {
            const dgq_gemm_conv_t& c = *p.ex.conv;
            DGQ_CHECK_ARG(c.codes_in && c.pixsum && c.pixsum_parts >= 1 && c.fill && a.per_m && a.L == 1 && a.w_bits == 4 && c.C > 0 && c.C % 16 == 0 && c.ldc >= c.C &&
                          c.ldc % 16 == 0 && c.kh >= 1 && c.kw >= 1 && c.stride >= 1 && c.Ho > 0 && c.Wo > 0 && c.B > 0 &&
                          a.M == c.B * c.Ho * c.Wo && a.Kp >= c.C * c.kh * c.kw && a.Kp - c.C * c.kh * c.kw < DGQ_KTILE + 16 &&
                          (reinterpret_cast<uintptr_t>(c.codes_in) & 15) == 0 && (reinterpret_cast<uintptr_t>(c.fill) & 15) == 0,
                          "dgq_gemm_wxa8: bad implicit-conv descriptor (needs per_m with L = 1, W4, C %% 16 == 0, M = B*Ho*Wo, 16-byte aligned codes_in / fill)");
            p.cv = c;
        }
        DGQ_CHECK_ARG(!p.ex.y2 || (p.ex.ldy2 >= a.N && !p.ex.geglu), "dgq_gemm_wxa8: y2 (second copy of the output rows) needs ldy2 >= N and no GEGLU epilogue");
        DGQ_CHECK_ARG(!p.ex.gn_partial || (a.M % 16 == 0 && a.N % 4 == 0 && !p.ex.geglu && p.ex.fq_mode == 0 &&
                                           (reinterpret_cast<uintptr_t>(p.ex.gn_partial) & 15) == 0),
                      "dgq_gemm_wxa8: GroupNorm partials need M %% 16 == 0, N %% 4 == 0, a 16-byte aligned buffer and no GEGLU / fused quantizer");
    } else {
        p.ex.residual = nullptr; p.ex.ldr = 0; p.ex.res_div = 1; p.ex.res_dtype = DGQ_F32; p.ex.fq_mode = 0; p.ex.fq_delta = nullptr; p.ex.fq_zp = nullptr;
        p.ex.fq_T = 1; p.ex.fq_D = 1; p.ex.fq_skip = 0; p.ex.fq_qmax = 255.0f; p.ex.geglu = 0; p.ex.gn_partial = nullptr; p.ex.conv = nullptr; p.ex.flush_coef = nullptr; p.ex.wfrag = nullptr; p.ex.act = nullptr;
        p.ex.y2 = nullptr; p.ex.ldy2 = 0;
    }
    p.splits = 1; p.slab = nullptr;
    p.tiles_per_split = a.Kp / BK;
    return DGQ_OK;
}

template <typename B>
static int dispatch_gemm(const B& bt, int w_bits, bool per_m, const GemmPlan& pl, int y_dtype, hipStream_t st) {
    if (w_bits == 4) return per_m ? launch_gemm<4, true>(bt, pl, y_dtype, st) : launch_gemm<4, false>(bt, pl, y_dtype, st);
    return per_m ? launch_gemm<8, true>(bt, pl, y_dtype, st) : launch_gemm<8, false>(bt, pl, y_dtype, st);
}

extern "C" int dgq_gemm_wxa8_batch(int n, const dgq_gemm_args_t* args, void* stream) {
    DGQ_CHECK_ARG(args && n >= 1 && n <= DGQ_GEMM_BATCH, "dgq_gemm_wxa8_batch: n=%d (1..%d)", n, DGQ_GEMM_BATCH);
    GemmBatch bt;
    bt.n = n;
    for (int i = 0; i < n; ++i) {
        const int rc = fill_gemm(args[i], bt.p[i]);
        if (rc != DGQ_OK) return rc;
        DGQ_CHECK_ARG(!bt.p[i].cv.codes_in, "dgq_gemm_wxa8_batch: implicit-conv problems take dgq_gemm_wxa8");
        DGQ_CHECK_ARG(args[i].w_bits == args[0].w_bits && (args[i].per_m != 0) == (args[0].per_m != 0) && args[i].y_dtype == args[0].y_dtype,
                      "dgq_gemm_wxa8_batch: problem %d differs from problem 0 in weight bits / scale mode / output dtype", i);
    }
    const dgq_gemm_args_t& a0 = args[0];
    GemmPlan pl = plan_gemm(a0.M, a0.N, a0.Kp, a0.w_bits, 0, a0.per_m != 0, n == 1);
    const bool fuse = bt.p[0].act.x != nullptr;
    for (int i = 1; i < n; ++i) DGQ_CHECK_ARG((bt.p[i].act.x != nullptr) == fuse, "dgq_gemm_wxa8_batch: quantise-on-load for all problems of a launch or none");
    if (fuse) {
        int maxKp = 0;
        for (int i = 0; i < n; ++i) maxKp = args[i].Kp > maxKp ? args[i].Kp : maxKp;
        DGQ_CHECK_ARG(plan_panel_fuse(a0.M, a0.N, maxKp, a0.per_m != 0, pl), "dgq_gemm_wxa8_batch: this shape does not take quantise-on-load (dgq_gemm_act_fuses)");
        GemmPlan f = pl;
        if (forced_plan(f) && f.fuse) pl = f;
    } else {
        forced_plan(pl);
        DGQ_CHECK_ARG(!pl.fuse, "dgq_gemm_wxa8_batch: DGQ_GEMM_FORCE names quantise-on-load, the call carries codes");
    }
    pl.splits = 1;
    return dispatch_gemm(bt, a0.w_bits, a0.per_m != 0, pl, a0.y_dtype, (hipStream_t)stream);
}

extern "C" int dgq_gemm_wxa8(const int8_t* codes, const float* rowsum, int rowsum_parts, int M, int Kp,
                             const void* wpacked, int w_bits, int N,
                             int per_m, const float* cdelta, const uint8_t* cflush,
                             const float* mdelta, const float* mzp, int L, float offset,
                             const float* alpha, const float* zw, const float* gamma, const float* vn,
                             void* y, int y_dtype, int ldy, void* workspace, size_t workspace_bytes,
                             const dgq_gemm_extra_t* extra, void* stream) {
    DGQ_CHECK_ARG(!workspace || (reinterpret_cast<uintptr_t>(workspace) & 15) == 0, "dgq_gemm_wxa8: workspace alignment");
    dgq_gemm_args_t a;
    a.codes = codes; a.rowsum = rowsum; a.rowsum_parts = rowsum_parts; a.M = M; a.Kp = Kp; a.wpacked = wpacked; a.w_bits = w_bits; a.N = N;
    a.per_m = per_m; a.cdelta = cdelta; a.cflush = cflush; a.mdelta = mdelta; a.mzp = mzp; a.L = L; a.offset = offset;
    a.alpha = alpha; a.zw = zw; a.gamma = gamma; a.vn = vn; a.y = y; a.y_dtype = y_dtype; a.ldy = ldy; a.extra = extra;
    GemmBatch bt;
    bt.n = 1;
    GemmParams& p = bt.p[0];
    const int rc = fill_gemm(a, p);
    if (rc != DGQ_OK) return rc;
    GemmPlan pl = plan_gemm(M, N, Kp, w_bits, workspace ? workspace_bytes : 0, per_m != 0, !p.cv.codes_in);
    if (p.act.x && p.act.kh > 1) {
        const dgq_gemm_act_t& q = p.act;
        int lds = 0;
        const int slab = dgq_gemm_convq_plan(q.B, q.H, q.W, q.K, q.kh, q.kw, q.stride, q.pad, N, Kp, w_bits, per_m != 0, &lds);
        const int Ho = (q.H + 2 * q.pad - q.kh) / q.stride + 1, Wo = (q.W + 2 * q.pad - q.kw) / q.stride + 1;
        DGQ_CHECK_ARG(slab > 0 && !p.cv.codes_in && M == q.B * Ho * Wo && !p.ex.geglu && p.ex.fq_mode == 0 && q.rows_per_image == q.H * q.W,
                      "dgq_gemm_wxa8: this convolution does not take quantise-on-load (dgq_gemm_conv_act_fuses)");
        p.splits = 1; p.slab = nullptr; p.tiles_per_split = Kp / BK;
        const int rc2 = dgq_launch_gemm_convq(bt, per_m != 0, y_dtype, slab, lds, (hipStream_t)stream);
        if (rc2 != DGQ_OK) return rc2;
        return dgq_launch_status("dgq_gemm_wxa8");
    }
    if (p.act.x) {
        DGQ_CHECK_ARG(!p.cv.codes_in && plan_panel_fuse(M, N, Kp, per_m != 0, pl), "dgq_gemm_wxa8: this shape does not take quantise-on-load (dgq_gemm_act_fuses)");
        GemmPlan f = pl;
        if (forced_plan(f) && f.fuse) pl = f;
        p.splits = 1; p.slab = nullptr; p.tiles_per_split = Kp / BK;
        return dispatch_gemm(bt, w_bits, per_m != 0, pl, y_dtype, (hipStream_t)stream);
    }
    if (p.cv.codes_in) {
        conv_tile(pl, M);
        const int thr = 256;
        hipLaunchKernelGGL(conv_rowsum_kernel, dim3((M + thr - 1) / thr), dim3(thr), 0, (hipStream_t)stream, p.cv, M, const_cast<float*>(rowsum));
        p.rowsum_parts = 1;
    }
    if (forced_plan(pl)) {
        DGQ_CHECK_ARG(!pl.fuse, "dgq_gemm_wxa8: DGQ_GEMM_FORCE names quantise-on-load, the call carries codes");
        if (p.cv.codes_in) { const int fs = pl.splits; conv_tile(pl, 0); pl.splits = fs; }
        DGQ_CHECK_ARG(pl.splits == 1 || (workspace && (size_t)pl.splits * M * N * 4 <= workspace_bytes),
                      "dgq_gemm_wxa8: DGQ_GEMM_FORCE split does not fit the workspace");
    }
    if (p.ex.geglu) pl.splits = 1;
    p.splits = pl.splits;
    p.slab = p.splits > 1 ? reinterpret_cast<float*>(workspace) : nullptr;
    const int nk = Kp / BK;
    p.tiles_per_split = (nk + p.splits - 1) / p.splits;
    p.splits = (nk + p.tiles_per_split - 1) / p.tiles_per_split;
    if (p.splits == 1) p.slab = nullptr;
    return dispatch_gemm(bt, w_bits, per_m != 0, pl, y_dtype, (hipStream_t)stream);
}
```

### dgq_amd/csrc/gemm_wxa8_big.hip

```cpp
#include "gemm_tile.h"

#ifndef BIG_GROUP_M
#define BIG_GROUP_M 4
#endif
#ifndef BIG_NPH_M
#define BIG_NPH_M 2
#endif
#ifndef BIG_NPH_K
#define BIG_NPH_K 1
#endif
#ifndef BIG_DMA_LOAD_M
#define BIG_DMA_LOAD_M 0
#endif
#ifndef BIG_DMA_LOAD_K
#define BIG_DMA_LOAD_K 0
#endif
#ifndef BIG_PRIO
#define BIG_PRIO 1
#endif

#ifndef BIG_PERK_TILE
#define BIG_PERK_TILE 1
#endif
#ifndef BIG_ABL
#define BIG_ABL 0
#endif

#ifndef BIG_STAMP
#define BIG_STAMP 0
#endif
#if !defined(DGQ_DIAG) && (BIG_ABL != 0 || BIG_STAMP != 0)
#error "BIG_ABL / BIG_STAMP change the kernel's results: diagnostic builds only (add -DDGQ_DIAG)"
#endif

namespace {

__device__ __forceinline__ uint64_t big_stamp() {
    uint64_t v;
    asm volatile("s_memtime %0\n\ts_waitcnt lgkmcnt(0)" : "=s"(v)::"memory");
    return v;
}

constexpr int BIG_WVM = 2, BIG_WVN = 4, BIG_NW = 8, BIG_NT = 512;

template <bool PER_M, typename TOut, int BM, int BN, int NBUF>
__global__ __launch_bounds__(BIG_NT, 2) void gemm_big_kernel(GemmBatch bt) {
    const GemmParams& p = bt.p[0];
    const uint64_t st_entry = BIG_STAMP == 2 ? big_stamp() : 0;
    int tile_n, tile_m;
    {
        const int gx = gridDim.x;
        const int logical = dgq_xcd_logical(blockIdx.x + gx * blockIdx.y, gx * gridDim.y);
        if (BIG_GROUP_M > 0) {
            constexpr int GM = BIG_GROUP_M > 0 ? BIG_GROUP_M : 1;
            const int gy = gridDim.y, band = logical / (GM * gx), first_m = band * GM;
            const int gsz = min(GM, gy - first_m), in = logical - band * GM * gx;
            tile_n = in / gsz;
            tile_m = first_m + (in - tile_n * gsz);
        } else {
            tile_m = logical / gx;
            tile_n = logical - tile_m * gx;
        }
    }
    extern __shared__ __attribute__((aligned(16))) uint8_t smem[];
    constexpr int WVM = BIG_WVM, WVN = BIG_WVN, NW = BIG_NW, NT = BIG_NT;
    constexpr int WM = BM / WVM, WN = BN / WVN;
    constexpr int TM = WM / 32, TN = WN / 32;
    constexpr int A_BYTES = BM * BK, W_ROW = BK / 2, W_BYTES = BN * W_ROW, STAGE_BYTES = A_BYTES + W_BYTES;
    constexpr int A_DMA = A_BYTES / 1024 / NW, W_DMA = W_BYTES / 1024 / NW, PER_TILE = A_DMA + W_DMA;
    static_assert(A_BYTES % (1024 * NW) == 0 && W_BYTES % (1024 * NW) == 0, "whole 1-KiB pieces per wave");
    static_assert(PER_TILE * 2 <= 63, "vmcnt is 6 bits");
    constexpr int NPH = PER_M ? BIG_NPH_M : BIG_NPH_K, CPP = NCH / NPH;

    const int tid = threadIdx.x;
    const int lane = tid & 63;
    const int wid = __builtin_amdgcn_readfirstlane(tid >> 6);
    const int group = wid >> 2;
    const int wave_m = wid >> 2, wave_n = wid & 3;
    const int n0 = tile_n * BN, m0 = tile_m * BM;
    const int nk = p.Kp / BK;

    const int8_t* a_src[A_DMA];
#pragma unroll
    for (int i = 0; i < A_DMA; ++i) {
        const int row = (wid * A_DMA + i) * 8 + (lane >> 3);
        const int c = (lane & 7) ^ ((row >> 1) & 7);
        a_src[i] = p.codes + (int64_t)min(m0 + row, p.M - 1) * p.Kp + 16 * c;
    }
    const uint8_t* w_src[W_DMA];
#pragma unroll
    for (int i = 0; i < W_DMA; ++i) {
        const int row = (wid * W_DMA + i) * 16 + (lane >> 2);
        const int c = (lane & 3) ^ ((row >> 2) & 3);
        w_src[i] = p.wpacked + (int64_t)min(n0 + row, p.N - 1) * (p.Kp / 2) + 16 * c;
    }
    const uint32_t lds_base = (uint32_t)(uintptr_t)(lptr_t)smem;
    auto issue_piece = [&](int q, int kt, int stage) {
        const uint32_t sa = lds_base + stage * STAGE_BYTES;
#pragma unroll
        for (int i = 0; i < A_DMA; ++i)
            if (q == i) glds16(a_src[i] + (int64_t)kt * BK, __builtin_amdgcn_readfirstlane(sa + (wid * A_DMA + i) * 1024));
#pragma unroll
        for (int i = 0; i < W_DMA; ++i)
            if (q == A_DMA + i) glds16(w_src[i] + (int64_t)kt * (BK / 2), __builtin_amdgcn_readfirstlane(sa + A_BYTES + (wid * W_DMA + i) * 1024));
    };

    v16i acc[TM][TN];
    v16f accf[TM][TN];
    constexpr bool BIASED = !PER_M;
    constexpr int ACC0 = BIASED ? DGQ_ACC_BIAS_I : 0;
#pragma unroll
    for (int i = 0; i < TM; ++i)
#pragma unroll
        for (int j = 0; j < TN; ++j)
#pragma unroll
            for (int r = 0; r < 16; ++r) { acc[i][j][r] = ACC0; accf[i][j][r] = 0.0f; }

    const int lr = lane & 31, hh = lane >> 5;
    int a_base[NCH], w_base[NCH];
    {
        const int ra = wave_m * WM + lr, rw = wave_n * WN + lr;
#pragma unroll
        for (int c = 0; c < NCH; ++c) {
            a_base[c] = ra * BK + (((2 * c + hh) ^ ((ra >> 1) & 7)) << 4);
            w_base[c] = rw * W_ROW + ((c ^ ((rw >> 2) & 3)) << 4) + ((hh ^ ((rw >> 4) & 1)) << 3);
        }
    }

    float* vtab = reinterpret_cast<float*>(smem + NBUF * STAGE_BYTES);
    float* vcol = vtab + 3 * BM;
    float* ctab = vcol + 4 * BN;
    static_assert(BM <= NT && BN <= NT, "one row / column of the epilogue vectors per thread");
#pragma unroll
    for (int q = 0; q < PER_TILE; ++q) issue_piece(q, 0, 0);
    if (nk > 1) {
#pragma unroll
        for (int q = 0; q < PER_TILE; ++q) issue_piece(q, 1, 1);
    }
    {
        if (tid < BM) {
            const int m = min(m0 + tid, p.M - 1);
            float rs = 0.0f;
            for (int j = 0; j < p.rowsum_parts; ++j) rs += p.rowsum[(int64_t)j * p.M + m];
            float r0 = 1.0f, r1 = rs, r2 = 0.0f;
            if (PER_M) {
                const int li = m % p.L;
                const float md = p.mdelta[li], mz = p.mzp[li];
                r0 = md; r1 = md * rs; r2 = md * (p.offset - mz);
            }
            vtab[tid] = r0; vtab[BM + tid] = r1; vtab[2 * BM + tid] = r2;
        }
        if (tid < BN) {
            const int n = min(n0 + tid, p.N - 1);
            vcol[tid] = p.alpha[n]; vcol[BN + tid] = p.zw[n]; vcol[2 * BN + tid] = p.gamma[n];
            vcol[3 * BN + tid] = PER_M ? p.vn[n] : 0.0f;
        }
        if constexpr (!PER_M) {
            const int nchunk = nk * NCH;
            const FlushGeom fg = {1, 0, nk, nk, 0};
#pragma unroll 1
            for (int e = tid; e < nchunk + nk; e += NT)
                ctab[e] = flush_entry(flush_ref(fg, e < nchunk, e < nchunk ? e : 0, e - nchunk), p.cdelta, p.cflush);
        }
    }
    asm volatile("s_waitcnt vmcnt(0) lgkmcnt(0)" ::: "memory");
    __builtin_amdgcn_s_barrier();
    if (group == 1) __builtin_amdgcn_s_barrier();

    const bool use_ccoef = !PER_M && p.ccoef != nullptr;
    const uint64_t st_loop0 = BIG_STAMP == 2 ? big_stamp() : 0;
    uint64_t stamps[6 * NPH];
    auto stamp = [&](int k, int t) {
        if (BIG_STAMP && t == 8) stamps[k] = big_stamp();
    };
#pragma unroll
    for (int k = 0; k < 6 * NPH; ++k) stamps[k] = 0;
    int stage = 0, istage = 2 % NBUF;
    auto pieces_in_phase = [](int ph) constexpr { int n = 0; for (int q = 0; q < PER_TILE; ++q) n += ((q * NPH) / PER_TILE == ph); return n; };
    auto pieces_before_phase = [](int ph) constexpr { int n = 0; for (int q = 0; q < PER_TILE; ++q) n += ((q * NPH) / PER_TILE < ph); return n; };
    auto piece_rank = [](int q, int ph) constexpr { int n = 0; for (int r = 0; r < q; ++r) n += ((r * NPH) / PER_TILE == ph); return n; };
    constexpr int DMA_LOAD = PER_M ? BIG_DMA_LOAD_M : BIG_DMA_LOAD_K;
    auto tile = [&](int t, auto dma_c) {
        constexpr bool DMA = decltype(dma_c)::value && !(BIG_ABL & 1);
        const uint8_t* sa = smem + stage * STAGE_BYTES;
        const uint8_t* sw = sa + A_BYTES;
#pragma unroll
        for (int ph = 0; ph < NPH; ++ph) {
            stamp(6 * ph + 0, t);
            v4i af[CPP][TM];
            uint2 wf[CPP][TN];
#pragma unroll
            for (int cc = 0; cc < CPP; ++cc) {
                const int c = ph * CPP + cc;
                if (BIG_ABL & 2) {
#pragma unroll
                    for (int j = 0; j < TN; ++j) wf[cc][j] = make_uint2(lane + c, lane + j);
#pragma unroll
                    for (int i = 0; i < TM; ++i) af[cc][i] = (v4i){lane, c, i, t};
                } else {
#pragma unroll
                    for (int j = 0; j < TN; ++j) wf[cc][j] = *reinterpret_cast<const uint2*>(sw + w_base[c] + j * (32 * W_ROW));
#pragma unroll
                    for (int i = 0; i < TM; ++i) af[cc][i] = *reinterpret_cast<const v4i*>(sa + a_base[c] + i * (32 * BK));
                }
            }
            int cqb[CPP];
            int tclr_b = 0;
            v4i c4 = {0, 0, 0, 0};
            float cq[CPP];
            float tclr = 0.0f;
            if constexpr (!PER_M) {
                if (__builtin_expect(use_ccoef, 1)) {
                    const float* cp = p.ccoef + (t * NCH + ph * CPP);
                    if constexpr (CPP == 4) {
                        asm volatile("s_load_dwordx4 %0, %1, 0x0" : "=s"(c4) : "s"(cp) : "memory");
                    } else {
#pragma unroll
                        for (int cc = 0; cc < CPP; ++cc) asm volatile("s_load_dword %0, %1, 0x0" : "=s"(cqb[cc]) : "s"(cp + cc) : "memory");
                    }
                    if (ph == NPH - 1) asm volatile("s_load_dword %0, %1, 0x0" : "=s"(tclr_b) : "s"(p.ccoef + nk * NCH + t) : "memory");
                } else {
#pragma unroll
                    for (int cc = 0; cc < CPP; ++cc) cq[cc] = ctab[t * NCH + ph * CPP + cc];
                    if (ph == NPH - 1) tclr = ctab[nk * NCH + t];
                }
            }
            if (DMA) {
#pragma unroll
                for (int q = 0; q < PER_TILE; ++q)
                    if ((q * NPH) / PER_TILE == ph && piece_rank(q, ph) < DMA_LOAD) issue_piece(q, t + 2, istage);
            }
            stamp(6 * ph + 1, t);
            if (ph == NPH - 1) {
                constexpr int YOUNGER = pieces_before_phase(NPH - 1) + (pieces_in_phase(NPH - 1) < DMA_LOAD ? pieces_in_phase(NPH - 1) : DMA_LOAD);
                if (DMA) asm volatile("s_waitcnt vmcnt(%0) lgkmcnt(0)" ::"n"(YOUNGER) : "memory");
                else asm volatile("s_waitcnt vmcnt(0) lgkmcnt(0)" ::: "memory");
            } else {
                asm volatile("s_waitcnt lgkmcnt(0)" ::: "memory");
            }
            if constexpr (!PER_M) {
                if (__builtin_expect(!use_ccoef, 0)) {
#pragma unroll
                    for (int cc = 0; cc < CPP; ++cc) cqb[cc] = __builtin_amdgcn_readfirstlane(__builtin_bit_cast(int, cq[cc]));
                    tclr_b = __builtin_amdgcn_readfirstlane(__builtin_bit_cast(int, tclr));
                } else {
                    if constexpr (CPP == 4) {
                        asm volatile("" : "+s"(c4), "+s"(tclr_b));
                        cqb[0] = c4.x; cqb[1] = c4.y; cqb[2] = c4.z; cqb[3] = c4.w;
                    } else {
#pragma unroll
                        for (int cc = 0; cc < CPP; ++cc) asm volatile("" : "+s"(cqb[cc]));
                        asm volatile("" : "+s"(tclr_b));
                    }
                }
            }
            v4i bf[CPP][TN];
#pragma unroll
            for (int cc = 0; cc < CPP; ++cc)
#pragma unroll
                for (int j = 0; j < TN; ++j) {
                    const uint2 v = wf[cc][j];
                    if (BIG_ABL & 4) bf[cc][j] = (v4i){(int)v.x, (int)v.y, (int)v.x, (int)v.y};
                    else bf[cc][j] = (v4i){(int)(v.x & 0x0F0F0F0Fu), (int)((v.x >> 4) & 0x0F0F0F0Fu),
                                           (int)(v.y & 0x0F0F0F0Fu), (int)((v.y >> 4) & 0x0F0F0F0Fu)};
                }
            stamp(6 * ph + 2, t);
            __builtin_amdgcn_sched_barrier(0);
            __builtin_amdgcn_s_barrier();
            stamp(6 * ph + 3, t);
            __builtin_amdgcn_sched_barrier(0);
            if (BIG_PRIO == 1) __builtin_amdgcn_s_setprio(1);
#pragma unroll
            for (int cc = 0; cc < CPP; ++cc) {
#pragma unroll
                for (int j = 0; j < TN; ++j)
#pragma unroll
                    for (int i = 0; i < TM; ++i)
                        acc[i][j] = __builtin_amdgcn_mfma_i32_32x32x32_i8(af[cc][i], bf[cc][j], acc[i][j], 0, 0, 0);
                if (DMA) {
#pragma unroll
                    for (int q = 0; q < PER_TILE; ++q)
                        if ((q * NPH) / PER_TILE == ph && piece_rank(q, ph) >= DMA_LOAD && (piece_rank(q, ph) - DMA_LOAD) % CPP == cc)
                            issue_piece(q, t + 2, istage);
                }
                if constexpr (!PER_M && !(BIG_ABL & 8)) {
                    if (__builtin_expect((cqb[cc] & 0x7FFFFFFF) != 0, 0)) {
                        const float sc = __builtin_bit_cast(float, cqb[cc]);
#pragma unroll
                        for (int j = 0; j < TN; ++j)
#pragma unroll
                            for (int i = 0; i < TM; ++i)
#pragma unroll
                                for (int r = 0; r < 16; ++r) accf[i][j][r] = __builtin_fmaf(sc, dgq_total_to_float<BIASED>(acc[i][j][r]), accf[i][j][r]);
                    }
                }
            }
            if constexpr (!PER_M) {
                if (ph == NPH - 1 && __builtin_expect(tclr_b != 0, 0)) {
#pragma unroll
                    for (int j = 0; j < TN; ++j)
#pragma unroll
                        for (int i = 0; i < TM; ++i)
#pragma unroll
                            for (int r = 0; r < 16; ++r) acc[i][j][r] = ACC0;
                }
            }
            if (BIG_PRIO == 1) __builtin_amdgcn_s_setprio(0);
            stamp(6 * ph + 4, t);
            __builtin_amdgcn_sched_barrier(0);
            __builtin_amdgcn_s_barrier();
            stamp(6 * ph + 5, t);
            __builtin_amdgcn_sched_barrier(0);
        }
        stage = (stage + 1 == NBUF) ? 0 : stage + 1;
        istage = (istage + 1 == NBUF) ? 0 : istage + 1;
    };
    int t = 0;
    for (; t + 2 < nk; ++t) tile(t, std::true_type());
    for (; t < nk; ++t) tile(t, std::false_type());
    if (group == 0) __builtin_amdgcn_s_barrier();
    const uint64_t st_loop1 = BIG_STAMP == 2 ? big_stamp() : 0;

    DGQ_DIAG_DECL
    gemm_store_tile<PER_M, TOut, BM, BN, WVM, WVN, 1, NBUF * STAGE_BYTES, TM, TN>(p, 0, smem, vtab, vcol, wid, lane, wave_m, wave_n, 0,
                                                                                  m0, n0, acc, accf DGQ_DIAG_ARG);
    const uint64_t st_issued = BIG_STAMP == 2 ? big_stamp() : 0;
    if (BIG_STAMP) {
        asm volatile("s_waitcnt vmcnt(0)" ::: "memory");
        __builtin_amdgcn_s_barrier();
    }
    if (BIG_STAMP == 2 && lane == 0 && blockIdx.y == 0 && (blockIdx.x == 0 || blockIdx.x == 8)) {
        uint64_t* dbg = reinterpret_cast<uint64_t*>(p.y) + (blockIdx.x ? 128 : 0) + wid * 16;
        dbg[0] = st_entry; dbg[1] = st_loop0; dbg[2] = st_loop1; dbg[3] = st_issued; dbg[4] = big_stamp();
        return;
    }
    if (BIG_STAMP && blockIdx.x == 0 && blockIdx.y == 0 && lane == 0) {
        uint64_t* dbg = reinterpret_cast<uint64_t*>(p.y) + wid * 16;
#pragma unroll
        for (int k = 0; k < 6 * NPH; ++k) dbg[k] = stamps[k];
    }
}

template <bool PER_M, typename TOut, int BM, int BN, int NBUF>
void launch_big(const GemmBatch& bt, hipStream_t st) {
    const GemmParams& p = bt.p[0];
    constexpr int stage = BM * BK + BN * (BK / 2);
    const int nk = p.Kp / BK;
    const int lds = NBUF * stage + (3 * BM + 4 * BN) * 4 + (PER_M ? 0 : (((NCH + 1) * nk * 4 + 15) & ~15));
    static std::atomic<bool> attr_set[64];
    dgq_allow_dynamic_lds(attr_set, {{&gemm_big_kernel<PER_M, TOut, BM, BN, NBUF>, 160 * 1024}});
    dim3 grid((p.N + BN - 1) / BN, (p.M + BM - 1) / BM, 1), block(BIG_NT);
    hipLaunchKernelGGL((gemm_big_kernel<PER_M, TOut, BM, BN, NBUF>), grid, block, lds, st, bt);
}

template <typename TOut>
int launch_big_dtype(const GemmBatch& bt, bool per_m, hipStream_t st) {
    if (per_m) launch_big<true, TOut, 256, 256, 3>(bt, st);
    else if (BIG_PERK_TILE == 0) launch_big<false, TOut, 128, 256, 3>(bt, st);
    else launch_big<false, TOut, 256, 128, 3>(bt, st);
    return DGQ_OK;
}

}

size_t dgq_gemm_big_lds_bytes(bool per_m, int Kp) {
    const int nk = Kp / BK;
    const int bm = (per_m || BIG_PERK_TILE) ? 256 : 128, bn = (per_m || !BIG_PERK_TILE) ? 256 : 128;
    return (size_t)3 * (bm * BK + bn * (BK / 2)) + (3 * bm + 4 * bn) * 4 + (per_m ? 0 : (((NCH + 1) * nk * 4 + 15) & ~15));
}

int dgq_launch_gemm_big(const GemmBatch& bt, bool per_m, int y_dtype, hipStream_t st) {
    switch (y_dtype) {
        case DGQ_F32: return launch_big_dtype<float>(bt, per_m, st);
        case DGQ_F16: return launch_big_dtype<__half>(bt, per_m, st);
        case DGQ_BF16: return launch_big_dtype<__hip_bfloat16>(bt, per_m, st);
        default: dgq_set_error("dgq_gemm_wxa8: unknown y dtype %d", y_dtype); return DGQ_EINVAL;
    }
}
```

### dgq_amd/csrc/linear_smallm.hip

```cpp
#include <atomic>
#include "dgq_common.h"
#include "gemm_device.h"

#define SMALLM_MAX_PROBLEMS 24
#define SMALLM_MAX_M 16
#define SMALLM_MAX_K 2048

struct SmallMProblem {
    const uint8_t* wpacked;
    const float* alpha;
    const float* zw;
    const float* gamma;
    const float* vn;
    const float* mdelta;
    const float* mzp;
    void* y;
    int ldy, N, Kp, w_bits, a_bits, block0;
};

struct SmallMBatch {
    SmallMProblem p[SMALLM_MAX_PROBLEMS];
    int n;
    const void* x;
    int x_dtype, y_dtype, M, K, ldx, pre_act;
};

template <typename TIn, typename TOut>
__global__ __launch_bounds__(256) void linear_smallm_kernel(SmallMBatch b) {
    extern __shared__ __attribute__((aligned(16))) uint8_t smem[];
    int pi = 0;
    while (pi + 1 < b.n && (int)blockIdx.x >= b.p[pi + 1].block0) ++pi;
    const SmallMProblem& P = b.p[pi];
    const int n0 = ((int)blockIdx.x - P.block0) * 64;
    const int tid = threadIdx.x, lane = tid & 63, wid = tid >> 6;
    const int Kq = (b.K + 15) & ~15;
    int8_t* codes = reinterpret_cast<int8_t*>(smem);
    const size_t codes_bytes = ((size_t)b.M * Kq + 15) & ~(size_t)15;
    float* rsum = reinterpret_cast<float*>(smem + codes_bytes);
    const float md = P.mdelta[0], mz = P.mzp[0], inv = dgq_rcp(md);
    const float qmax = (float)((1 << P.a_bits) - 1), off = (float)(1 << (P.a_bits - 1));
    if (tid < b.M) rsum[tid] = 0.0f;
    __syncthreads();
    const TIn* x = reinterpret_cast<const TIn*>(b.x);
    for (int m = 0; m < b.M; ++m) {
        float part = 0.0f;
        for (int k = tid; k < Kq; k += 256) {
            float c = 0.0f;
            if (k < b.K) {
                float v = dgq_to_float(x[(int64_t)m * b.ldx + k]);
                if (b.pre_act == 1) v = dgq_silu(v);
                c = dgq_affine_code_fast(v, md, inv, mz, qmax) - off;
            }
            codes[m * Kq + k] = (int8_t)(int)c;
            part += c;
        }
#pragma unroll
        for (int o = 32; o > 0; o >>= 1) part += __shfl_xor(part, o, 64);
        if (lane == 0) atomicAdd(&rsum[m], part);
    }
    __syncthreads();
    TOut* y = reinterpret_cast<TOut*>(P.y);
    const int row_bytes = P.w_bits == 4 ? P.Kp / 2 : P.Kp;
    if (P.w_bits == 4) {
        const int k0 = lane * 32;
        const bool live = k0 < Kq;
        uint4 wq[16];
#pragma unroll
        for (int r = 0; r < 16; ++r) {
            const int n = min(n0 + wid * 16 + r, P.N - 1);
            wq[r] = live ? *reinterpret_cast<const uint4*>(P.wpacked + (int64_t)n * row_bytes + k0 / 2) : make_uint4(0u, 0u, 0u, 0u);
        }
        int* red = reinterpret_cast<int*>(smem + codes_bytes + 64) + wid * (32 * 65);
        for (int m0 = 0; m0 < b.M; m0 += 2) {
            int4 c0[2], c1[2];
#pragma unroll
            for (int mm = 0; mm < 2; ++mm) {
                const int m = min(m0 + mm, b.M - 1);
                c0[mm] = live ? *reinterpret_cast<const int4*>(codes + m * Kq + k0) : make_int4(0, 0, 0, 0);
                c1[mm] = (live && k0 + 16 < Kq) ? *reinterpret_cast<const int4*>(codes + m * Kq + k0 + 16) : make_int4(0, 0, 0, 0);
            }
#pragma unroll
            for (int r = 0; r < 16; ++r) {
                const bool sw = ((n0 + wid * 16 + r) & 16) != 0;
                const uint4 w = wq[r];
                const unsigned ww[4] = {sw ? w.z : w.x, sw ? w.w : w.y, sw ? w.x : w.z, sw ? w.y : w.w};
#pragma unroll
                for (int mm = 0; mm < 2; ++mm) {
                    const int cc[8] = {c0[mm].x, c0[mm].y, c0[mm].z, c0[mm].w, c1[mm].x, c1[mm].y, c1[mm].z, c1[mm].w};
                    int a = 0;
#pragma unroll
                    for (int j = 0; j < 4; ++j) {
                        a = __builtin_amdgcn_sdot4(cc[2 * j], (int)(ww[j] & 0x0F0F0F0Fu), a, false);
                        a = __builtin_amdgcn_sdot4(cc[2 * j + 1], (int)((ww[j] >> 4) & 0x0F0F0F0Fu), a, false);
                    }
                    red[(2 * r + mm) * 65 + lane] = a;
                }
            }
            asm volatile("s_waitcnt lgkmcnt(0)" ::: "memory");
            if (lane < 32) {
                int tot = 0;
#pragma unroll 16
                for (int l = 0; l < 64; ++l) tot += red[lane * 65 + l];
                const int r = lane >> 1, m = m0 + (lane & 1), n = n0 + wid * 16 + r;
                if (m < b.M && n < P.N) {
                    const float rs = rsum[m];
                    const float out = dgq_dequant<true>((float)tot, md, md * rs, md * (off - mz), P.alpha[n], P.zw[n], P.gamma[n], P.vn[n]);
                    y[(int64_t)m * P.ldy + n] = dgq_from_float<TOut>(out);
                }
            }
            asm volatile("s_waitcnt lgkmcnt(0)" ::: "memory");
        }
        return;
    }
    for (int r = 0; r < 16; ++r) {
        const int n = n0 + wid * 16 + r;
        if (n >= P.N) break;
        const uint8_t* wrow = P.wpacked + (int64_t)n * row_bytes;
        int acc[SMALLM_MAX_M];
#pragma unroll
        for (int m = 0; m < SMALLM_MAX_M; ++m) acc[m] = 0;
        for (int k0 = lane * 16; k0 < Kq; k0 += 64 * 16) {
            const int4 w = *reinterpret_cast<const int4*>(wrow + k0);
#pragma unroll
            for (int m = 0; m < SMALLM_MAX_M; ++m) {
                if (m >= b.M) continue;
                const int4 c = *reinterpret_cast<const int4*>(codes + m * Kq + k0);
                int a = acc[m];
                a = __builtin_amdgcn_sdot4(c.x, w.x, a, false);
                a = __builtin_amdgcn_sdot4(c.y, w.y, a, false);
                a = __builtin_amdgcn_sdot4(c.z, w.z, a, false);
                a = __builtin_amdgcn_sdot4(c.w, w.w, a, false);
                acc[m] = a;
            }
        }
        const float al = P.alpha[n], zw = P.zw[n], ga = P.gamma[n], vn = P.vn[n];
#pragma unroll
        for (int m = 0; m < SMALLM_MAX_M; ++m) {
            if (m >= b.M) continue;
            int a = acc[m];
#pragma unroll
            for (int o = 32; o > 0; o >>= 1) a += __shfl_xor(a, o, 64);
            if (lane == 0) {
                const float rs = rsum[m];
                const float out = dgq_dequant<true>((float)a, md, md * rs, md * (off - mz), al, zw, ga, vn);
                y[(int64_t)m * P.ldy + n] = dgq_from_float<TOut>(out);
            }
        }
    }
}

extern "C" int dgq_linear_smallm_batch(const void* x, int x_dtype, int M, int K, int64_t ldx, int pre_act, int n_problems,
                                       const dgq_smallm_problem_t* probs, int y_dtype, void* stream) {
    DGQ_CHECK_ARG(x && probs, "dgq_linear_smallm_batch: null pointer");
    DGQ_CHECK_ARG(M >= 1 && M <= SMALLM_MAX_M && K >= 1 && K <= SMALLM_MAX_K && ldx >= K, "dgq_linear_smallm_batch: M=%d (<= %d) K=%d (<= %d)", M, SMALLM_MAX_M, K, SMALLM_MAX_K);
    DGQ_CHECK_ARG(n_problems >= 1 && n_problems <= SMALLM_MAX_PROBLEMS, "dgq_linear_smallm_batch: %d problems (max %d)", n_problems, SMALLM_MAX_PROBLEMS);
    DGQ_CHECK_ARG(pre_act == 0 || pre_act == 1, "dgq_linear_smallm_batch: pre_act");
    SmallMBatch b;
    b.n = n_problems; b.x = x; b.x_dtype = x_dtype; b.y_dtype = y_dtype; b.M = M; b.K = K; b.ldx = (int)ldx; b.pre_act = pre_act;
    int blocks = 0;
    for (int i = 0; i < n_problems; ++i) {
        const dgq_smallm_problem_t& q = probs[i];
        DGQ_CHECK_ARG(q.wpacked && q.alpha && q.zw && q.gamma && q.vn && q.mdelta && q.mzp && q.y, "dgq_linear_smallm_batch: null pointer in problem %d", i);
        DGQ_CHECK_ARG(q.N > 0 && q.ldy >= q.N && q.Kp >= K && q.Kp % DGQ_KTILE == 0 && (q.w_bits == 4 || q.w_bits == 8) && q.a_bits >= 2 && q.a_bits <= 8,
                      "dgq_linear_smallm_batch: bad problem %d", i);
        DGQ_CHECK_ARG((reinterpret_cast<uintptr_t>(q.wpacked) & 15) == 0, "dgq_linear_smallm_batch: wpacked alignment");
        SmallMProblem& P = b.p[i];
        P.wpacked = reinterpret_cast<const uint8_t*>(q.wpacked); P.alpha = q.alpha; P.zw = q.zw; P.gamma = q.gamma; P.vn = q.vn;
        P.mdelta = q.mdelta; P.mzp = q.mzp; P.y = q.y; P.ldy = q.ldy; P.N = q.N; P.Kp = q.Kp; P.w_bits = q.w_bits; P.a_bits = q.a_bits;
        P.block0 = blocks;
        blocks += (q.N + 63) / 64;
    }
    const size_t lds = ((((size_t)M * ((K + 15) & ~15)) + 15) & ~(size_t)15) + 64 + 4 * (32 * 65) * sizeof(int);
    static std::atomic<bool> attr_set[64];
    dgq_allow_dynamic_lds(attr_set, {{&linear_smallm_kernel<float, float>, 72 * 1024},
                                     {&linear_smallm_kernel<__half, __half>, 72 * 1024},
                                     {&linear_smallm_kernel<__hip_bfloat16, __hip_bfloat16>, 72 * 1024}});
    hipStream_t st = (hipStream_t)stream;
#define DGQ_SMALLM(TI, TO) hipLaunchKernelGGL((linear_smallm_kernel<TI, TO>), dim3(blocks), dim3(256), lds, st, b)
    if (x_dtype == DGQ_F32 && y_dtype == DGQ_F32) DGQ_SMALLM(float, float);
    else if (x_dtype == DGQ_F16 && y_dtype == DGQ_F16) DGQ_SMALLM(__half, __half);
    else if (x_dtype == DGQ_BF16 && y_dtype == DGQ_BF16) DGQ_SMALLM(__hip_bfloat16, __hip_bfloat16);
    else { dgq_set_error("dgq_linear_smallm_batch: x/y dtypes %d/%d", x_dtype, y_dtype); return DGQ_EINVAL; }
#undef DGQ_SMALLM
    return dgq_launch_status("dgq_linear_smallm_batch");
}
```

Before: 121.2 steps/s.

## Add LDS-staged tiled small-N conv, single-stage small-K conv, and prefetching small-M linear

Adds a spatially tiled small-N fp32-weight conv kernel that stages the input patch and the weights in LDS once per workgroup. It is selected by default and can be disabled through an env var. Also adds a small-K conv kernel that loads the whole K range in one pass and writes output through an LDS transpose as vectorised stores. The small-M linear kernel now prefetches activations and weights before quantisation, uses an unrolled problem lookup, and hoists per-column dequant params. This spreads several unrelated changes across multiple files, raising LDS use and register pressure and adding complexity.

```diff
diff --git a/dgq_amd/csrc/conv_f32w.hip b/dgq_amd/csrc/conv_f32w.hip
--- a/dgq_amd/csrc/conv_f32w.hip
+++ b/dgq_amd/csrc/conv_f32w.hip
@@ -1,6 +1,9 @@
+#include <atomic>
+#include <cstdlib>
 #include "quant_common.h"
 
 typedef float v16f __attribute__((ext_vector_type(16)));
+typedef float v4f __attribute__((ext_vector_type(4)));
 
 struct ConvF32Params {
     const void* x;
@@ -40,6 +43,33 @@
 #define CF_BN 64
 #define CF_BK 16
 #define CF_LD (CF_BK + 1)
+
+__device__ __forceinline__ void conv_f32w_gn_partials(const ConvF32Params& p, const v16f& acc, float bias, int lane, int mw, int n) {
+#pragma unroll
+    for (int blk = 0; blk < 2; ++blk) {
+        float val[8], sum = 0.0f;
+#pragma unroll
+        for (int q = 0; q < 8; ++q) {
+            float v = acc[blk * 8 + q] + bias;
+            if (p.y_dtype == DGQ_F16) v = __half2float(__float2half(v));
+            else if (p.y_dtype == DGQ_BF16) v = __bfloat162float(__float2bfloat16(v));
+            val[q] = v;
+            sum += v;
+        }
+        float mean = sum * 0.125f, m2 = 0.0f;
+#pragma unroll
+        for (int q = 0; q < 8; ++q) m2 += (val[q] - mean) * (val[q] - mean);
+        const float om = __shfl_xor(mean, 32, 64), o2 = __shfl_xor(m2, 32, 64);
+        const float dd = om - mean;
+        m2 = m2 + o2 + dd * dd * 4.0f;
+        mean = 0.5f * (mean + om);
+        const int mb = mw + blk * 16;
+        if ((lane >> 5) == 0 && mb < p.M) {
+            float* q2 = p.gn_partial + ((int64_t)(mb >> 4) * p.N + n) * 2;
+            q2[0] = mean; q2[1] = m2;
+        }
+    }
+}
 
 __global__ __launch_bounds__(256) void conv_f32w_kernel(ConvF32Params p) {
     __shared__ float As[CF_BM][CF_LD];
@@ -98,32 +128,101 @@
         store_any(p.y, p.y_dtype, (int64_t)m * p.ldy + n, v);
         if (p.y2) store_any(p.y2, p.y_dtype, (int64_t)m * p.ldy2 + n, v);
     }
-    if (p.gn_partial) {
-#pragma unroll
-        for (int blk = 0; blk < 2; ++blk) {
-            float val[8], sum = 0.0f;
-#pragma unroll
-            for (int q = 0; q < 8; ++q) {
-                float v = acc[blk * 8 + q] + bias;
-                if (p.y_dtype == DGQ_F16) v = __half2float(__float2half(v));
-                else if (p.y_dtype == DGQ_BF16) v = __bfloat162float(__float2bfloat16(v));
-                val[q] = v;
-                sum += v;
-            }
-            float mean = sum * 0.125f, m2 = 0.0f;
-#pragma unroll
-            for (int q = 0; q < 8; ++q) m2 += (val[q] - mean) * (val[q] - mean);
-            const float om = __shfl_xor(mean, 32, 64), o2 = __shfl_xor(m2, 32, 64);
-            const float dd = om - mean;
-            m2 = m2 + o2 + dd * dd * 4.0f;
-            mean = 0.5f * (mean + om);
-            const int mb = m0 + wm + blk * 16;
-            if ((lane >> 5) == 0 && mb < p.M) {
-                float* q2 = p.gn_partial + ((int64_t)(mb >> 4) * p.N + n) * 2;
-                q2[0] = mean; q2[1] = m2;
-            }
-        }
-    }
+    if (p.gn_partial) conv_f32w_gn_partials(p, acc, bias, lane, m0 + wm, n);
+}
+
+#define CF_KS 48
+#define CF_LDK (CF_KS + 1)
+#define CF_LDT (CF_BN + 4)
+__global__ __launch_bounds__(256) void conv_f32w_smallk_kernel(ConvF32Params p, int rc, int rkw, int vec_store) {
+    __shared__ __attribute__((aligned(16))) float sm[2 * CF_BM * CF_LDK];
+    static_assert(CF_BM * CF_LDT <= 2 * CF_BM * CF_LDK && CF_BM == CF_BN, "the output tile reuses the operand tiles");
+    float (*As)[CF_LDK] = reinterpret_cast<float (*)[CF_LDK]>(sm);
+    float (*Bs)[CF_LDK] = reinterpret_cast<float (*)[CF_LDK]>(sm + CF_BM * CF_LDK);
+    const int tid = threadIdx.x, lane = tid & 63, wid = tid >> 6;
+    const int m0 = blockIdx.y * CF_BM, n0 = blockIdx.x * CF_BN;
+    const int wm = (wid >> 1) * 32, wn = (wid & 1) * 32;
+    const int srow = tid >> 2, sk = (tid & 3) * 4;
+    const bool a_live = m0 + srow < p.M, b_live = n0 + srow < p.N;
+    const int am = min(m0 + srow, p.M - 1), bn = min(n0 + srow, p.N - 1);
+    const int L = p.Ho * p.Wo;
+    const int ab = am / L, l = am - ab * L;
+    const int aho = l / p.Wo, awo = l - aho * p.Wo;
+    const int Kpad = (p.K + CF_BK - 1) & ~(CF_BK - 1);
+    float a[12], bw[12];
+#pragma unroll
+    for (int e = 0; e < 12; ++e) {
+        const int k = (e >> 2) * CF_BK + sk + (e & 3), kc = min(k, p.K - 1);
+        const int tap = (kc * rc) >> 16, c = kc - tap * p.C;
+        const int dh = (tap * rkw) >> 16, dw = tap - dh * p.kw;
+        const int hi = aho * p.stride - p.pad + dh, wi = awo * p.stride - p.pad + dw;
+        const bool inb = k < p.K && a_live && hi >= 0 && hi < p.H && wi >= 0 && wi < p.W;
+        const int hc = min(max(hi, 0), p.H - 1), wc = min(max(wi, 0), p.W - 1);
+        const float av = ld_pre(p, ab, ((int64_t)ab * p.H + hc) * p.W + wc, c);
+        const float bv = p.w[(int64_t)bn * p.K + kc];
+        a[e] = inb ? av : 0.0f;
+        bw[e] = (k < p.K && b_live) ? bv : 0.0f;
+    }
+#pragma unroll
+    for (int e = 0; e < 12; ++e) {
+        As[srow][(e >> 2) * CF_BK + sk + (e & 3)] = a[e];
+        Bs[srow][(e >> 2) * CF_BK + sk + (e & 3)] = bw[e];
+    }
+    __syncthreads();
+    v16f acc;
+#pragma unroll
+    for (int r = 0; r < 16; ++r) acc[r] = 0.0f;
+    for (int k0 = 0; k0 < Kpad; k0 += CF_BK) {
+#pragma unroll
+        for (int kk = 0; kk < CF_BK; kk += 2) {
+            const float av = As[wm + (lane & 31)][k0 + kk + (lane >> 5)];
+            const float bv = Bs[wn + (lane & 31)][k0 + kk + (lane >> 5)];
+            acc = __builtin_amdgcn_mfma_f32_32x32x2f32(av, bv, acc, 0, 0, 0);
+        }
+    }
+    const int n = n0 + wn + (lane & 31);
+    const float bias = p.bias ? p.bias[min(n, p.N - 1)] : 0.0f;
+    if (vec_store) {
+        float (*Ts)[CF_LDT] = reinterpret_cast<float (*)[CF_LDT]>(sm);
+        __syncthreads();
+#pragma unroll
+        for (int r = 0; r < 16; ++r) Ts[wm + (r & 3) + 8 * (r >> 2) + 4 * (lane >> 5)][wn + (lane & 31)] = acc[r] + bias;
+        __syncthreads();
+#pragma unroll
+        for (int i = 0; i < 4; ++i) {
+            const int row = (tid >> 4) + 16 * i, col = (tid & 15) * 4;
+            const int m = m0 + row, nn = n0 + col;
+            if (m >= p.M || nn >= p.N) continue;
+            const float4 v = *reinterpret_cast<const float4*>(&Ts[row][col]);
+            if (p.y_dtype == DGQ_F32) {
+                *reinterpret_cast<float4*>(reinterpret_cast<float*>(p.y) + (int64_t)m * p.ldy + nn) = v;
+                if (p.y2) *reinterpret_cast<float4*>(reinterpret_cast<float*>(p.y2) + (int64_t)m * p.ldy2 + nn) = v;
+            } else {
+                uint2 t;
+                if (p.y_dtype == DGQ_F16) {
+                    const __half h[4] = {__float2half(v.x), __float2half(v.y), __float2half(v.z), __float2half(v.w)};
+                    t = *reinterpret_cast<const uint2*>(h);
+                } else {
+                    const __hip_bfloat16 h[4] = {__float2bfloat16(v.x), __float2bfloat16(v.y), __float2bfloat16(v.z), __float2bfloat16(v.w)};
+                    t = *reinterpret_cast<const uint2*>(h);
+                }
+                *reinterpret_cast<uint2*>(reinterpret_cast<uint16_t*>(p.y) + (int64_t)m * p.ldy + nn) = t;
+                if (p.y2) *reinterpret_cast<uint2*>(reinterpret_cast<uint16_t*>(p.y2) + (int64_t)m * p.ldy2 + nn) = t;
+            }
+        }
+    }
+    if (n >= p.N) return;
+    if (!vec_store) {
+#pragma unroll
+        for (int r = 0; r < 16; ++r) {
+            const int m = m0 + wm + (r & 3) + 8 * (r >> 2) + 4 * (lane >> 5);
+            if (m >= p.M) continue;
+            const float v = acc[r] + bias;
+            store_any(p.y, p.y_dtype, (int64_t)m * p.ldy + n, v);
+            if (p.y2) store_any(p.y2, p.y_dtype, (int64_t)m * p.ldy2 + n, v);
+        }
+    }
+    if (p.gn_partial) conv_f32w_gn_partials(p, acc, bias, lane, m0 + wm, n);
 }
 
 template <int NMAX>
@@ -208,6 +307,166 @@
             if (p.y2) store_any(p.y2, p.y_dtype, (int64_t)m * p.ldy2 + n, v);
         }
     }
+}
+
+#define CF_TILE_NT 512
+#define CF_TILE_NW (CF_TILE_NT / 64)
+#define CF_TILE_PPW 4
+template <int NMAX, typename TIn, bool PRE>
+__global__ __launch_bounds__(CF_TILE_NT) void conv_f32w_smalln_tiled_kernel(ConvF32Params p, int TH, int TW) {
+    extern __shared__ __attribute__((aligned(16))) float cf_lds[];
+    const int tid = threadIdx.x, lane = tid & 63, wid = tid >> 6;
+    const int PH = (TH - 1) * p.stride + p.kh, PW = (TW - 1) * p.stride + p.kw;
+    const int tiles_w = (p.Wo + TW - 1) / TW, tiles_h = (p.Ho + TH - 1) / TH;
+    const int b = blockIdx.x / (tiles_h * tiles_w), tr = blockIdx.x - b * (tiles_h * tiles_w);
+    const int ho0 = (tr / tiles_w) * TH, wo0 = (tr % tiles_w) * TW;
+    const int c4n = p.C >> 2;
+    float* patch = cf_lds;
+    float* wl = cf_lds + PH * PW * p.C;
+    constexpr int WR = 6, PR = 10;
+    const int n4 = (p.N * p.K) >> 2, n_el = PH * PW * c4n;
+    const int hb = ho0 * p.stride - p.pad, wb = wo0 * p.stride - p.pad;
+    v4f wv[WR];
+    float4 v[PR], sc[PR], sh[PR];
+    bool inb[PR];
+    auto w_issue = [&](int i0) __attribute__((always_inline)) {
+#pragma unroll
+        for (int j = 0; j < WR; ++j) wv[j] = *reinterpret_cast<const v4f*>(p.w + 4 * (int64_t)min(i0 + CF_TILE_NT * j, n4 - 1));
+    };
+    auto w_commit = [&](int i0) __attribute__((always_inline)) {
+#pragma unroll
+        for (int j = 0; j < WR; ++j)
+            if (i0 + CF_TILE_NT * j < n4) *reinterpret_cast<v4f*>(wl + 4 * (i0 + CF_TILE_NT * j)) = wv[j];
+    };
+    auto patch_issue = [&](int i0) __attribute__((always_inline)) {
+#pragma unroll
+        for (int j = 0; j < PR; ++j) {
+            const int i = min(i0 + CF_TILE_NT * j, n_el - 1);
+            const int pix = i / c4n, c = (i - pix * c4n) << 2;
+            const int ph = pix / PW, pw = pix - ph * PW;
+            const int hi = hb + ph, wi = wb + pw;
+            inb[j] = hi >= 0 && hi < p.H && wi >= 0 && wi < p.W;
+            const int hc = min(max(hi, 0), p.H - 1), wc = min(max(wi, 0), p.W - 1);
+            const int64_t xi = (((int64_t)b * p.H + hc) * p.W + wc) * p.C + c;
+            float t4[4];
+            load4<TIn>(reinterpret_cast<const TIn*>(p.x) + xi, t4);
+            v[j] = make_float4(t4[0], t4[1], t4[2], t4[3]);
+            if constexpr (PRE) {
+                sc[j] = *reinterpret_cast<const float4*>(p.pre_scale + (int64_t)b * p.C + c);
+                sh[j] = *reinterpret_cast<const float4*>(p.pre_shift + (int64_t)b * p.C + c);
+            }
+        }
+    };
+    auto patch_commit = [&](int i0) __attribute__((always_inline)) {
+#pragma unroll
+        for (int j = 0; j < PR; ++j) {
+            float4 t = v[j];
+            if constexpr (PRE) {
+                t.x = t.x * sc[j].x + sh[j].x; t.y = t.y * sc[j].y + sh[j].y; t.z = t.z * sc[j].z + sh[j].z; t.w = t.w * sc[j].w + sh[j].w;
+            }
+            if (p.pre_act == 1) { t.x = dgq_silu(t.x); t.y = dgq_silu(t.y); t.z = dgq_silu(t.z); t.w = dgq_silu(t.w); }
+            if (!inb[j]) t = make_float4(0.0f, 0.0f, 0.0f, 0.0f);
+            if (i0 + CF_TILE_NT * j < n_el) *reinterpret_cast<float4*>(patch + 4 * (i0 + CF_TILE_NT * j)) = t;
+        }
+    };
+    w_issue(tid);
+    patch_issue(tid);
+    patch_commit(tid);
+    w_commit(tid);
+    for (int i0 = tid + CF_TILE_NT * PR; i0 < n_el; i0 += CF_TILE_NT * PR) { patch_issue(i0); patch_commit(i0); }
+    for (int i0 = tid + CF_TILE_NT * WR; i0 < n4; i0 += CF_TILE_NT * WR) { w_issue(i0); w_commit(i0); }
+    __syncthreads();
+    const int npos = TH * TW;
+    int pbase[CF_TILE_PPW];
+    bool plive[CF_TILE_PPW];
+    int64_t prow[CF_TILE_PPW];
+#pragma unroll
+    for (int q = 0; q < CF_TILE_PPW; ++q) {
+        const int pos = min(wid + CF_TILE_NW * q, npos - 1);
+        const int lh = pos / TW, lw = pos - lh * TW;
+        plive[q] = (wid + CF_TILE_NW * q < npos) && (ho0 + lh < p.Ho) && (wo0 + lw < p.Wo);
+        pbase[q] = (lh * p.stride * PW + lw * p.stride) * p.C;
+        prow[q] = ((int64_t)b * p.Ho + (ho0 + lh)) * p.Wo + (wo0 + lw);
+    }
+    const int nq = min(CF_TILE_PPW, (npos - wid + CF_TILE_NW - 1) / CF_TILE_NW);
+    float acc[CF_TILE_PPW][NMAX];
+#pragma unroll
+    for (int q = 0; q < CF_TILE_PPW; ++q)
+#pragma unroll
+        for (int n = 0; n < NMAX; ++n) acc[q][n] = 0.0f;
+    const int units = p.kh * p.kw * c4n;
+    constexpr int UB = NMAX <= 4 ? 4 : 2;
+    for (int u0 = lane; u0 < units; u0 += 64 * UB) {
+        float4 w4[UB][NMAX];
+        int uoff[UB];
+        bool ulive[UB];
+#pragma unroll
+        for (int j = 0; j < UB; ++j) {
+            const int u = min(u0 + 64 * j, units - 1);
+            const int tap = u / c4n, c = (u - tap * c4n) << 2;
+            const int dh = tap / p.kw, dw = tap - dh * p.kw;
+            ulive[j] = u0 + 64 * j < units;
+            uoff[j] = (dh * PW + dw) * p.C + c;
+#pragma unroll
+            for (int n = 0; n < NMAX; ++n)
+                if (n < p.N) w4[j][n] = *reinterpret_cast<const float4*>(wl + n * p.K + tap * p.C + c);
+        }
+#pragma unroll
+        for (int q = 0; q < CF_TILE_PPW; ++q) {
+            if (q >= nq) break;
+            float4 t[UB];
+#pragma unroll
+            for (int j = 0; j < UB; ++j) {
+                t[j] = *reinterpret_cast<const float4*>(patch + pbase[q] + uoff[j]);
+                if (!ulive[j]) t[j] = make_float4(0.0f, 0.0f, 0.0f, 0.0f);
+            }
+#pragma unroll
+            for (int j = 0; j < UB; ++j)
+#pragma unroll
+                for (int n = 0; n < NMAX; ++n)
+                    if (n < p.N) {
+                        acc[q][n] = __builtin_fmaf(t[j].x, w4[j][n].x, acc[q][n]);
+                        acc[q][n] = __builtin_fmaf(t[j].y, w4[j][n].y, acc[q][n]);
+                        acc[q][n] = __builtin_fmaf(t[j].z, w4[j][n].z, acc[q][n]);
+                        acc[q][n] = __builtin_fmaf(t[j].w, w4[j][n].w, acc[q][n]);
+                    }
+        }
+    }
+#pragma unroll
+    for (int q = 0; q < CF_TILE_PPW; ++q) {
+        if (q >= nq) break;
+#pragma unroll
+        for (int n = 0; n < NMAX; ++n) {
+            float v = acc[q][n];
+#pragma unroll
+            for (int o = 32; o > 0; o >>= 1) v += __shfl_xor(v, o, 64);
+            if (lane == 0 && n < p.N && plive[q]) {
+                v += p.bias ? p.bias[n] : 0.0f;
+                store_any(p.y, p.y_dtype, prow[q] * p.ldy + n, v);
+                if (p.y2) store_any(p.y2, p.y_dtype, prow[q] * p.ldy2 + n, v);
+            }
+        }
+    }
+}
+
+static bool conv_f32w_staged_forms() {
+    const char* e = getenv("DGQ_CONV_F32W_FORM");
+    return !(e && e[0] == '0' && e[1] == 0);
+}
+
+static bool conv_f32w_pick_tile(const ConvF32Params& p, int& TH, int& TW, size_t& lds) {
+    static const int cand[4][2] = {{4, 8}, {4, 4}, {2, 4}, {2, 2}};
+    bool found = false;
+    for (int i = 0; i < 4; ++i) {
+        const int th = cand[i][0], tw = cand[i][1];
+        const size_t PH = (size_t)(th - 1) * p.stride + p.kh, PW = (size_t)(tw - 1) * p.stride + p.kw;
+        const size_t bytes = (PH * PW * p.C + (size_t)p.N * p.K) * sizeof(float);
+        if (bytes > 160 * 1024) continue;
+        TH = th; TW = tw; lds = bytes; found = true;
+        const int64_t grid = (int64_t)p.B * ((p.Ho + th - 1) / th) * ((p.Wo + tw - 1) / tw);
+        if (grid >= 256) break;
+    }
+    return found;
 }
 
 extern "C" int dgq_conv2d_f32w(const void* x, int x_dtype, int B, int H, int W, int C, int kh, int kw, int stride, int pad,
@@ -229,13 +488,46 @@
     p.y2 = y2; p.ldy2 = ldy2;
     DGQ_CHECK_ARG(!gn_partial || (p.M % 16 == 0 && N > 8), "dgq_conv2d_f32w: GroupNorm partials need M %% 16 == 0 and the tiled kernel (N > 8)");
     p.gn_partial = gn_partial;
+    const bool staged = conv_f32w_staged_forms();
     if (N <= 8) {
+        const bool vec = (C & 3) == 0 && ((reinterpret_cast<uintptr_t>(x) | reinterpret_cast<uintptr_t>(w)) & 15) == 0 &&
+                         (!pre_scale || ((reinterpret_cast<uintptr_t>(pre_scale) | reinterpret_cast<uintptr_t>(pre_shift)) & 15) == 0);
+        int TH = 0, TW = 0;
+        size_t lds = 0;
+        if (staged && vec && conv_f32w_pick_tile(p, TH, TW, lds)) {
+            const int64_t grid = (int64_t)B * ((p.Ho + TH - 1) / TH) * ((p.Wo + TW - 1) / TW);
+            DGQ_CHECK_ARG(grid <= 0x7fffffff, "dgq_conv2d_f32w: %lld workgroups exceed the grid", (long long)grid);
+            static std::atomic<bool> attr_set[64];
+#define DGQ_CF_TILED(NM, TI) {&conv_f32w_smalln_tiled_kernel<NM, TI, false>, 160 * 1024}, {&conv_f32w_smalln_tiled_kernel<NM, TI, true>, 160 * 1024}
+            dgq_allow_dynamic_lds(attr_set, {DGQ_CF_TILED(4, float), DGQ_CF_TILED(8, float), DGQ_CF_TILED(4, __half), DGQ_CF_TILED(8, __half),
+                                             DGQ_CF_TILED(4, __hip_bfloat16), DGQ_CF_TILED(8, __hip_bfloat16)});
+#undef DGQ_CF_TILED
+            const hipStream_t st = (hipStream_t)stream;
+            auto launch = [&](auto tin) {
+                typedef decltype(tin) TI;
+                if (N <= 4 && pre_scale) hipLaunchKernelGGL((conv_f32w_smalln_tiled_kernel<4, TI, true>), dim3((unsigned)grid), dim3(CF_TILE_NT), lds, st, p, TH, TW);
+                else if (N <= 4) hipLaunchKernelGGL((conv_f32w_smalln_tiled_kernel<4, TI, false>), dim3((unsigned)grid), dim3(CF_TILE_NT), lds, st, p, TH, TW);
+                else if (pre_scale) hipLaunchKernelGGL((conv_f32w_smalln_tiled_kernel<8, TI, true>), dim3((unsigned)grid), dim3(CF_TILE_NT), lds, st, p, TH, TW);
+                else hipLaunchKernelGGL((conv_f32w_smalln_tiled_kernel<8, TI, false>), dim3((unsigned)grid), dim3(CF_TILE_NT), lds, st, p, TH, TW);
+            };
+            if (x_dtype == DGQ_F32) launch(float());
+            else if (x_dtype == DGQ_F16) launch(__half());
+            else launch(__hip_bfloat16());
+            return dgq_launch_status("dgq_conv2d_f32w");
+        }
         if (N <= 4) hipLaunchKernelGGL(conv_f32w_smalln_kernel<4>, dim3((p.M + 3) / 4), dim3(256), 0, (hipStream_t)stream, p);
         else hipLaunchKernelGGL(conv_f32w_smalln_kernel<8>, dim3((p.M + 3) / 4), dim3(256), 0, (hipStream_t)stream, p);
         return dgq_launch_status("dgq_conv2d_f32w");
     }
     dim3 grid((N + CF_BN - 1) / CF_BN, (p.M + CF_BM - 1) / CF_BM);
     DGQ_CHECK_ARG(grid.y <= 65535, "dgq_conv2d_f32w: M = %d rows exceed the grid", p.M);
+    if (staged && p.K <= CF_KS) {
+        const size_t es = y_dtype == DGQ_F32 ? 4 : 2;
+        auto rows_aligned = [&](const void* q, int ld) { return (reinterpret_cast<uintptr_t>(q) % (4 * es)) == 0 && (ld & 3) == 0; };
+        const int vec_store = (N & 3) == 0 && rows_aligned(y, ldy) && (!y2 || rows_aligned(y2, ldy2));
+        hipLaunchKernelGGL(conv_f32w_smallk_kernel, grid, dim3(256), 0, (hipStream_t)stream, p, (65536 + C - 1) / C, (65536 + kw - 1) / kw, vec_store);
+        return dgq_launch_status("dgq_conv2d_f32w");
+    }
     hipLaunchKernelGGL(conv_f32w_kernel, grid, dim3(256), 0, (hipStream_t)stream, p);
     return dgq_launch_status("dgq_conv2d_f32w");
 }
diff --git a/dgq_amd/csrc/gemm_tile.h b/dgq_amd/csrc/gemm_tile.h
--- a/dgq_amd/csrc/gemm_tile.h
+++ b/dgq_amd/csrc/gemm_tile.h
@@ -54,11 +54,40 @@
                  "s"(p.ex.res_div), "s"(p.ex.res_dtype), "s"(p.ex.fq_mode), "s"(p.ex.geglu), "s"(p.ex.gn_partial), "s"(p.wfrag), "s"(p.ex.y2));
 }
 
+#define DGQ_ROWSUM_ROUND 16
+template <int R>
+__device__ __forceinline__ void gemm_rowsum_issue(float (&v)[R], const float* rowsum, int jb, int parts, int M, int m) {
+#pragma unroll
+    for (int j = 0; j < R; ++j) v[j] = rowsum[(int64_t)min(jb + j, parts - 1) * M + m];
+}
+template <int R>
+__device__ __forceinline__ float gemm_rowsum_fold(float rs, const float (&v)[R], int jb, int parts) {
+#pragma unroll
+    for (int j = 0; j < R; ++j)
+        if (jb + j < parts) rs += v[j];
+    return rs;
+}
+template <int R>
+__device__ __forceinline__ float gemm_rowsum_rounds(float rs, const float* rowsum, int j0, int parts, int M, int m) {
+    for (int jb = j0; jb < parts; jb += R) {
+        float v[R];
+        gemm_rowsum_issue<R>(v, rowsum, jb, parts, M, m);
+        rs = gemm_rowsum_fold<R>(rs, v, jb, parts);
+    }
+    return rs;
+}
+__device__ __forceinline__ float gemm_rowsum_add(float rs, const float* rowsum, int j0, int parts, int M, int m) {
+    const int n = parts - j0;
+    if (n <= 0) return rs;
+    if (n == 1) return rs + rowsum[(int64_t)j0 * M + m];
+    if (n <= 4) return gemm_rowsum_rounds<4>(rs, rowsum, j0, parts, M, m);
+    return gemm_rowsum_rounds<DGQ_ROWSUM_ROUND>(rs, rowsum, j0, parts, M, m);
+}
+
 template <bool PER_M>
 __device__ __forceinline__ float dgq_epilogue(const GemmParams& p, float acc, int m, int n, float al, float zw, float ga,
                                               float vn) {
-    float rs = 0.0f;
-    for (int j = 0; j < p.rowsum_parts; ++j) rs += p.rowsum[(int64_t)j * p.M + m];
+    const float rs = gemm_rowsum_add(0.0f, p.rowsum, 0, p.rowsum_parts, p.M, m);
     if (PER_M) {
         const int li = m % p.L;
         const float md = p.mdelta[li], mz = p.mzp[li];
diff --git a/dgq_amd/csrc/gemm_wxa8.hip b/dgq_amd/csrc/gemm_wxa8.hip
--- a/dgq_amd/csrc/gemm_wxa8.hip
+++ b/dgq_amd/csrc/gemm_wxa8.hip
@@ -342,6 +342,52 @@
     auto row4 = [&](int m, int nb, float (&val)[4], bool live) {
         float a[4] = {0.f, 0.f, 0.f, 0.f};
         const bool full = (nb + 3 < p.N) && ((p.N & 3) == 0);
+        if (full && vec4) {
+            const float4 al = *reinterpret_cast<const float4*>(p.alpha + nb), zw = *reinterpret_cast<const float4*>(p.zw + nb);
+            const float4 ga = *reinterpret_cast<const float4*>(p.gamma + nb);
+            const float4 vn = PER_M ? *reinterpret_cast<const float4*>(p.vn + nb) : make_float4(0.f, 0.f, 0.f, 0.f);
+            float md = 1.0f, mz = 0.0f;
+            if (PER_M) {
+                const int li = m % p.L;
+                md = p.mdelta[li]; mz = p.mzp[li];
+            }
+            float r[4] = {0.f, 0.f, 0.f, 0.f};
+            if (p.ex.residual) {
+                const int64_t ri = (int64_t)(m / p.ex.res_div) * p.ex.ldr + nb;
+                if (p.ex.res_dtype == DGQ_F32) load4<float>(reinterpret_cast<const float*>(p.ex.residual) + ri, r);
+                else if (p.ex.res_dtype == DGQ_BF16) load4<__hip_bfloat16>(reinterpret_cast<const __hip_bfloat16*>(p.ex.residual) + ri, r);
+                else load4<__half>(reinterpret_cast<const __half*>(p.ex.residual) + ri, r);
+            }
+            float pv[DGQ_ROWSUM_ROUND] = {};
+            if (p.rowsum_parts > 1) gemm_rowsum_issue<DGQ_ROWSUM_ROUND>(pv, p.rowsum, 0, p.rowsum_parts, p.M, m);
+            else pv[0] = p.rowsum[m];
+            splitk_sum(p.slab + (int64_t)m * p.N + nb, slab_stride, p.splits, a);
+            float rs = gemm_rowsum_fold<DGQ_ROWSUM_ROUND>(0.0f, pv, 0, p.rowsum_parts);
+            rs = gemm_rowsum_add(rs, p.rowsum, DGQ_ROWSUM_ROUND, p.rowsum_parts, p.M, m);
+            float r0 = 1.0f, r1 = rs, r2 = 0.0f;
+            if (PER_M) { r0 = md; r1 = md * rs; r2 = md * (p.offset - mz); }
+            float o[4];
+            o[0] = dgq_dequant<PER_M>(a[0], r0, r1, r2, al.x, zw.x, ga.x, vn.x);
+            o[1] = dgq_dequant<PER_M>(a[1], r0, r1, r2, al.y, zw.y, ga.y, vn.y);
+            o[2] = dgq_dequant<PER_M>(a[2], r0, r1, r2, al.z, zw.z, ga.z, vn.z);
+            o[3] = dgq_dequant<PER_M>(a[3], r0, r1, r2, al.w, zw.w, ga.w, vn.w);
+            if (p.ex.residual) { o[0] += r[0]; o[1] += r[1]; o[2] += r[2]; o[3] += r[3]; }
+            TOut* dst = y + (int64_t)m * p.ldy + nb;
+            TOut* dst2 = p.ex.y2 ? reinterpret_cast<TOut*>(p.ex.y2) + (int64_t)m * p.ex.ldy2 + nb : nullptr;
+            if (sizeof(TOut) == 4) {
+                if (live) *reinterpret_cast<float4*>(dst) = make_float4(o[0], o[1], o[2], o[3]);
+                if (live && dst2) *reinterpret_cast<float4*>(dst2) = make_float4(o[0], o[1], o[2], o[3]);
+#pragma unroll
+                for (int e = 0; e < 4; ++e) val[e] = o[e];
+            } else {
+                TOut t[4] = {dgq_from_float<TOut>(o[0]), dgq_from_float<TOut>(o[1]), dgq_from_float<TOut>(o[2]), dgq_from_float<TOut>(o[3])};
+                if (live) *reinterpret_cast<uint2*>(dst) = *reinterpret_cast<const uint2*>(t);
+                if (live && dst2) *reinterpret_cast<uint2*>(dst2) = *reinterpret_cast<const uint2*>(t);
+#pragma unroll
+                for (int e = 0; e < 4; ++e) val[e] = dgq_to_float(t[e]);
+            }
+            return;
+        }
         if (full) {
             splitk_sum(p.slab + (int64_t)m * p.N + nb, slab_stride, p.splits, a);
         } else {
@@ -349,47 +395,6 @@
                 const float* src = p.slab + s * slab_stride + (int64_t)m * p.N + nb;
                 for (int e = 0; e < 4 && nb + e < p.N; ++e) a[e] += src[e];
             }
-        }
-        if (full && vec4) {
-            const float4 al = *reinterpret_cast<const float4*>(p.alpha + nb), zw = *reinterpret_cast<const float4*>(p.zw + nb);
-            const float4 ga = *reinterpret_cast<const float4*>(p.gamma + nb);
-            const float4 vn = PER_M ? *reinterpret_cast<const float4*>(p.vn + nb) : make_float4(0.f, 0.f, 0.f, 0.f);
-            float rs = 0.0f;
-            for (int j = 0; j < p.rowsum_parts; ++j) rs += p.rowsum[(int64_t)j * p.M + m];
-            float r0 = 1.0f, r1 = rs, r2 = 0.0f;
-            if (PER_M) {
-                const int li = m % p.L;
-                const float md = p.mdelta[li], mz = p.mzp[li];
-                r0 = md; r1 = md * rs; r2 = md * (p.offset - mz);
-            }
-            float o[4];
-            o[0] = dgq_dequant<PER_M>(a[0], r0, r1, r2, al.x, zw.x, ga.x, vn.x);
-            o[1] = dgq_dequant<PER_M>(a[1], r0, r1, r2, al.y, zw.y, ga.y, vn.y);
-            o[2] = dgq_dequant<PER_M>(a[2], r0, r1, r2, al.z, zw.z, ga.z, vn.z);
-            o[3] = dgq_dequant<PER_M>(a[3], r0, r1, r2, al.w, zw.w, ga.w, vn.w);
-            if (p.ex.residual) {
-                const int64_t ri = (int64_t)(m / p.ex.res_div) * p.ex.ldr + nb;
-                float r[4];
-                if (p.ex.res_dtype == DGQ_F32) load4<float>(reinterpret_cast<const float*>(p.ex.residual) + ri, r);
-                else if (p.ex.res_dtype == DGQ_BF16) load4<__hip_bfloat16>(reinterpret_cast<const __hip_bfloat16*>(p.ex.residual) + ri, r);
-                else load4<__half>(reinterpret_cast<const __half*>(p.ex.residual) + ri, r);
-                o[0] += r[0]; o[1] += r[1]; o[2] += r[2]; o[3] += r[3];
-            }
-            TOut* dst = y + (int64_t)m * p.ldy + nb;
-            TOut* dst2 = p.ex.y2 ? reinterpret_cast<TOut*>(p.ex.y2) + (int64_t)m * p.ex.ldy2 + nb : nullptr;
-            if (sizeof(TOut) == 4) {
-                if (live) *reinterpret_cast<float4*>(dst) = make_float4(o[0], o[1], o[2], o[3]);
-                if (live && dst2) *reinterpret_cast<float4*>(dst2) = make_float4(o[0], o[1], o[2], o[3]);
-#pragma unroll
-                for (int e = 0; e < 4; ++e) val[e] = o[e];
-            } else {
-                TOut t[4] = {dgq_from_float<TOut>(o[0]), dgq_from_float<TOut>(o[1]), dgq_from_float<TOut>(o[2]), dgq_from_float<TOut>(o[3])};
-                if (live) *reinterpret_cast<uint2*>(dst) = *reinterpret_cast<const uint2*>(t);
-                if (live && dst2) *reinterpret_cast<uint2*>(dst2) = *reinterpret_cast<const uint2*>(t);
-#pragma unroll
-                for (int e = 0; e < 4; ++e) val[e] = dgq_to_float(t[e]);
-            }
-            return;
         }
         for (int e = 0; e < 4 && nb + e < p.N; ++e) {
             const int n = nb + e;
diff --git a/dgq_amd/csrc/gemm_wxa8_big.hip b/dgq_amd/csrc/gemm_wxa8_big.hip
--- a/dgq_amd/csrc/gemm_wxa8_big.hip
+++ b/dgq_amd/csrc/gemm_wxa8_big.hip
@@ -140,8 +140,7 @@
     {
         if (tid < BM) {
             const int m = min(m0 + tid, p.M - 1);
-            float rs = 0.0f;
-            for (int j = 0; j < p.rowsum_parts; ++j) rs += p.rowsum[(int64_t)j * p.M + m];
+            const float rs = gemm_rowsum_add(0.0f, p.rowsum, 0, p.rowsum_parts, p.M, m);
             float r0 = 1.0f, r1 = rs, r2 = 0.0f;
             if (PER_M) {
                 const int li = m % p.L;
diff --git a/dgq_amd/csrc/linear_smallm.hip b/dgq_amd/csrc/linear_smallm.hip
--- a/dgq_amd/csrc/linear_smallm.hip
+++ b/dgq_amd/csrc/linear_smallm.hip
@@ -1,4 +1,5 @@
 #include <atomic>
+#include <climits>
 #include "dgq_common.h"
 #include "gemm_device.h"
 
@@ -15,11 +16,12 @@
     const float* mdelta;
     const float* mzp;
     void* y;
-    int ldy, N, Kp, w_bits, a_bits, block0;
+    int ldy, N, Kp, w_bits, a_bits;
 };
 
 struct SmallMBatch {
     SmallMProblem p[SMALLM_MAX_PROBLEMS];
+    int block0[SMALLM_MAX_PROBLEMS];
     int n;
     const void* x;
     int x_dtype, y_dtype, M, K, ldx, pre_act;
@@ -28,48 +30,73 @@
 template <typename TIn, typename TOut>
 __global__ __launch_bounds__(256) void linear_smallm_kernel(SmallMBatch b) {
     extern __shared__ __attribute__((aligned(16))) uint8_t smem[];
-    int pi = 0;
-    while (pi + 1 < b.n && (int)blockIdx.x >= b.p[pi + 1].block0) ++pi;
+    int pi = 0, first = 0;
+#pragma unroll
+    for (int i = 1; i < SMALLM_MAX_PROBLEMS; ++i)
+        if ((int)blockIdx.x >= b.block0[i]) { pi = i; first = b.block0[i]; }
     const SmallMProblem& P = b.p[pi];
-    const int n0 = ((int)blockIdx.x - P.block0) * 64;
+    const int n0 = ((int)blockIdx.x - first) * 64;
     const int tid = threadIdx.x, lane = tid & 63, wid = tid >> 6;
     const int Kq = (b.K + 15) & ~15;
     int8_t* codes = reinterpret_cast<int8_t*>(smem);
     const size_t codes_bytes = ((size_t)b.M * Kq + 15) & ~(size_t)15;
     float* rsum = reinterpret_cast<float*>(smem + codes_bytes);
+    static_assert(256 * 8 >= SMALLM_MAX_K, "one round of eight k steps per thread covers a row");
+    const TIn* x = reinterpret_cast<const TIn*>(b.x);
+    TIn xv[2][8];
+    auto load_pair = [&](int m0) {
+#pragma unroll
+        for (int mm = 0; mm < 2; ++mm)
+#pragma unroll
+            for (int u = 0; u < 8; ++u)
+                xv[mm][u] = x[(int64_t)min(m0 + mm, b.M - 1) * b.ldx + min(tid + 256 * u, b.K - 1)];
+    };
+    load_pair(0);
+    const int row_bytes = P.w_bits == 4 ? P.Kp / 2 : P.Kp;
+    const int k0 = lane * 32;
+    const bool live = k0 < Kq;
+    uint4 wq[16];
+#pragma unroll
+    for (int r = 0; r < 16; ++r) {
+        const int n = min(n0 + wid * 16 + r, P.N - 1);
+        wq[r] = *reinterpret_cast<const uint4*>(P.wpacked + (int64_t)n * row_bytes + (live ? k0 / 2 : 0));
+    }
+    const int en = min(n0 + wid * 16 + ((lane & 31) >> 1), P.N - 1);
+    const float e_al = P.alpha[en], e_zw = P.zw[en], e_ga = P.gamma[en], e_vn = P.vn[en];
     const float md = P.mdelta[0], mz = P.mzp[0], inv = dgq_rcp(md);
     const float qmax = (float)((1 << P.a_bits) - 1), off = (float)(1 << (P.a_bits - 1));
     if (tid < b.M) rsum[tid] = 0.0f;
     __syncthreads();
-    const TIn* x = reinterpret_cast<const TIn*>(b.x);
-    for (int m = 0; m < b.M; ++m) {
-        float part = 0.0f;
-        for (int k = tid; k < Kq; k += 256) {
-            float c = 0.0f;
-            if (k < b.K) {
-                float v = dgq_to_float(x[(int64_t)m * b.ldx + k]);
-                if (b.pre_act == 1) v = dgq_silu(v);
-                c = dgq_affine_code_fast(v, md, inv, mz, qmax) - off;
-            }
-            codes[m * Kq + k] = (int8_t)(int)c;
-            part += c;
-        }
-#pragma unroll
-        for (int o = 32; o > 0; o >>= 1) part += __shfl_xor(part, o, 64);
-        if (lane == 0) atomicAdd(&rsum[m], part);
+    auto quant_pair = [&](int m0) {
+#pragma unroll
+        for (int mm = 0; mm < 2; ++mm) {
+            float part = 0.0f;
+#pragma unroll
+            for (int u = 0; u < 8; ++u) {
+                const int k = tid + 256 * u;
+                float t = dgq_to_float(xv[mm][u]);
+                if (b.pre_act == 1) t = dgq_silu(t);
+                float c = dgq_affine_code_fast(t, md, inv, mz, qmax) - off;
+                if (k >= b.K) c = 0.0f;
+                if (k < Kq && m0 + mm < b.M) codes[(m0 + mm) * Kq + k] = (int8_t)(int)c;
+                if (k < Kq) part += c;
+            }
+#pragma unroll
+            for (int o = 32; o > 0; o >>= 1) part += __shfl_xor(part, o, 64);
+            if (lane == 0 && m0 + mm < b.M) atomicAdd(&rsum[m0 + mm], part);
+        }
+    };
+    quant_pair(0);
+    for (int m0 = 2; m0 < b.M; m0 += 2) {
+        load_pair(m0);
+        quant_pair(m0);
     }
     __syncthreads();
     TOut* y = reinterpret_cast<TOut*>(P.y);
-    const int row_bytes = P.w_bits == 4 ? P.Kp / 2 : P.Kp;
     if (P.w_bits == 4) {
-        const int k0 = lane * 32;
-        const bool live = k0 < Kq;
-        uint4 wq[16];
-#pragma unroll
-        for (int r = 0; r < 16; ++r) {
-            const int n = min(n0 + wid * 16 + r, P.N - 1);
-            wq[r] = live ? *reinterpret_cast<const uint4*>(P.wpacked + (int64_t)n * row_bytes + k0 / 2) : make_uint4(0u, 0u, 0u, 0u);
-        }
+#pragma unroll
+        for (int r = 0; r < 16; ++r)
+            if (!live) wq[r] = make_uint4(0u, 0u, 0u, 0u);
         int* red = reinterpret_cast<int*>(smem + codes_bytes + 64) + wid * (32 * 65);
         for (int m0 = 0; m0 < b.M; m0 += 2) {
             int4 c0[2], c1[2];
@@ -104,7 +131,7 @@
                 const int r = lane >> 1, m = m0 + (lane & 1), n = n0 + wid * 16 + r;
                 if (m < b.M && n < P.N) {
                     const float rs = rsum[m];
-                    const float out = dgq_dequant<true>((float)tot, md, md * rs, md * (off - mz), P.alpha[n], P.zw[n], P.gamma[n], P.vn[n]);
+                    const float out = dgq_dequant<true>((float)tot, md, md * rs, md * (off - mz), e_al, e_zw, e_ga, e_vn);
                     y[(int64_t)m * P.ldy + n] = dgq_from_float<TOut>(out);
                 }
             }
@@ -158,6 +185,7 @@
     SmallMBatch b;
     b.n = n_problems; b.x = x; b.x_dtype = x_dtype; b.y_dtype = y_dtype; b.M = M; b.K = K; b.ldx = (int)ldx; b.pre_act = pre_act;
     int blocks = 0;
+    for (int i = n_problems; i < SMALLM_MAX_PROBLEMS; ++i) b.block0[i] = INT_MAX;
     for (int i = 0; i < n_problems; ++i) {
         const dgq_smallm_problem_t& q = probs[i];
         DGQ_CHECK_ARG(q.wpacked && q.alpha && q.zw && q.gamma && q.vn && q.mdelta && q.mzp && q.y, "dgq_linear_smallm_batch: null pointer in problem %d", i);
@@ -167,7 +195,7 @@
         SmallMProblem& P = b.p[i];
         P.wpacked = reinterpret_cast<const uint8_t*>(q.wpacked); P.alpha = q.alpha; P.zw = q.zw; P.gamma = q.gamma; P.vn = q.vn;
         P.mdelta = q.mdelta; P.mzp = q.mzp; P.y = q.y; P.ldy = q.ldy; P.N = q.N; P.Kp = q.Kp; P.w_bits = q.w_bits; P.a_bits = q.a_bits;
-        P.block0 = blocks;
+        b.block0[i] = blocks;
         blocks += (q.N + 63) / 64;
     }
     const size_t lds = ((((size_t)M * ((K + 15) & ~15)) + 15) & ~(size_t)15) + 64 + 4 * (32 * 65) * sizeof(int);
```

After: 122.1 steps/s, median of 6. About the same (+0.7%).
